# li-kunyi/CUT3R-SLAM

Hardware: AMD Instinct MI355X
Metric: frames/sec (ViT pointmap + covisibility-graph tracking step) on 640x480 (higher is better)
Workload: dtype f16

## Files before the change

cut3r_slam_amd/_lib.py:

```python
from __future__ import annotations

import ctypes as C
import os

_HERE = os.path.dirname(os.path.abspath(__file__))
LIB_PATH = os.path.join(_HERE, "libcut3r_hip.so")

c_void_p, c_int, c_float, c_ll = C.c_void_p, C.c_int, C.c_float, C.c_longlong


class GemmDesc(C.Structure):
    _fields_ = [
        ("A", c_void_p), ("B", c_void_p), ("C", c_void_p), ("bias", c_void_p), ("res1", c_void_p), ("res2", c_void_p),
        ("M", c_int), ("N", c_int), ("K", c_int), ("lda", c_int), ("ldb", c_int), ("ldc", c_int), ("ldr1", c_int),
        ("ldr2", c_int),
        ("act", c_int), ("out_f16", c_int), ("res1_f16", c_int), ("res2_f16", c_int),
        ("batch", c_int),
        ("strideA", c_ll), ("strideB", c_ll), ("strideC", c_ll), ("strideBias", c_ll), ("strideR1", c_ll),
        ("strideR2", c_ll),
        ("conv_k", c_int), ("H", c_int), ("W", c_int), ("Cin", c_int), ("conv_stride", c_int), ("Ho", c_int),
        ("Wo", c_int), ("relu_in", c_int),
        ("shuf", c_int), ("shuf_cout", c_int), ("shuf_Hin", c_int), ("shuf_Win", c_int),
        ("tile", c_int), ("stages", c_int),
        ("rope_pos", c_void_p), ("rope_table", c_void_p), ("rope_cols", c_int), ("rope_pmin", c_int), ("rope_npos", c_int),
        ("rope_d", c_int),
        ("ln_stats", c_void_p), ("ln_colsum", c_void_p), ("ln_nslab", c_int), ("ln_eps", c_float),
        ("stats_out", c_void_p), ("out16", c_void_p), ("ld16", c_int),
    ]


class LcTerm(C.Structure):
    _fields_ = [("a", c_void_p), ("c", c_void_p), ("mask", c_void_p), ("ia", c_int), ("ic", c_int), ("w", c_float), ("pad", c_int)]


SIGNATURES = {
    "cut3r_abi_version": [],
    "cut3r_rope2d": [c_void_p, c_int, c_void_p, c_int, c_int, c_int, c_int, c_ll, c_ll, c_ll, c_float, c_float, c_void_p],
    "cut3r_rope2d_qk": [c_void_p, c_void_p, c_int, c_void_p, c_int, c_int, c_int, c_int, c_ll, c_ll, c_ll, c_ll, c_float, c_float,
                        c_void_p],
    "cut3r_rope2d_tab": [c_void_p, c_void_p, c_ll, c_ll, c_void_p, c_void_p, c_ll, c_ll, c_int, c_int, c_void_p, c_int, c_int, c_float,
                         c_float, c_void_p],
    "cut3r_layernorm": [c_void_p, c_int, c_void_p, c_void_p, c_float, c_int, c_int, c_void_p, c_int, c_void_p, c_int,
                        c_void_p, c_void_p, c_void_p],
    "cut3r_layernorm_dual": [c_void_p, c_int, c_void_p, c_void_p, c_void_p, c_int, c_void_p, c_void_p, c_void_p, c_int, c_float, c_int,
                             c_int, c_void_p],
    "cut3r_layernorm_tokens": [c_void_p, c_int, c_void_p, c_void_p, c_float, c_int, c_int, c_int, c_void_p, c_ll, c_void_p, c_ll, c_void_p,
                               c_ll, c_void_p, c_ll, c_void_p],
    "cut3r_gemm_f16": [C.POINTER(GemmDesc), c_void_p],
    "cut3r_gemm_tile_for": [C.POINTER(GemmDesc)],
    "cut3r_gemm_f16_pair": [C.POINTER(GemmDesc), C.POINTER(GemmDesc), c_void_p],
    "cut3r_gemm_kernel_for": [C.POINTER(GemmDesc)],
    "cut3r_gemm_pair_kernel_for": [C.POINTER(GemmDesc), C.POINTER(GemmDesc)],
    "cut3r_gemm_kernel_count": [],
    "cut3r_rope2d_table": [c_void_p, c_int, c_int, c_int, c_float, c_float, c_void_p],
    "cut3r_gemv_f16w": [c_void_p, c_int, c_void_p, c_int, c_void_p, c_void_p, c_int, c_int, c_int, c_int, c_int,
                        c_void_p, c_int, c_int, c_void_p],
    "cut3r_attention_variant": [c_int],
    "cut3r_attention_kernel_for": [c_int, c_int, c_int, c_int],
    "cut3r_attention_f16": [c_void_p, c_void_p, c_void_p, c_void_p, c_int, c_int, c_int, c_int, c_int,
                            c_ll, c_ll, c_ll, c_ll, c_ll, c_ll, c_ll, c_ll, c_float, c_void_p],
    "cut3r_attention_one_key_f16": [c_void_p, c_void_p, c_int, c_int, c_int, c_int, c_ll, c_ll, c_ll, c_ll, c_void_p],
    "cut3r_im2col_patch": [c_void_p, c_int, c_int, c_int, c_int, c_int, c_int, c_void_p, c_void_p],
    "cut3r_cast_f32_f16": [c_void_p, c_int, c_void_p, c_int, c_int, c_int, c_void_p],
    "cut3r_colmean": [c_void_p, c_int, c_int, c_int, c_void_p, c_void_p],
    "cut3r_colmean_batched": [c_void_p, c_int, c_ll, c_int, c_int, c_int, c_void_p, c_ll, c_void_p],
    "cut3r_upsample2x_nhwc": [c_void_p, c_void_p, c_int, c_int, c_int, c_int, c_void_p],
    "cut3r_dpt_final": [c_void_p, c_int, c_int, c_void_p, c_void_p, c_int, c_void_p, c_void_p, c_void_p],
    "cut3r_conv3x3_dpt_final": [C.POINTER(GemmDesc), c_void_p, c_void_p, c_int, c_void_p, c_ll, c_void_p, c_ll, c_void_p],
    "cut3r_postprocess_pts": [c_void_p, c_int, c_int, c_int, c_void_p, c_void_p, c_void_p],
    "cut3r_postprocess_pose": [c_void_p, c_int, c_void_p, c_void_p],
    "cut3r_patch_overlap": [c_void_p, c_void_p, c_int, c_int, c_float, c_void_p, c_void_p, c_void_p],
    "cut3r_patch_overlap_chain": [c_void_p, c_void_p, c_int, c_int, c_int, c_float, C.c_double, c_void_p, c_void_p, c_void_p, c_void_p,
                                  c_void_p, c_void_p],
    "cut3r_overlap_fwd": [c_void_p, c_int, C.POINTER(c_float), c_float, c_void_p, c_int, c_float, c_float, c_float, c_float,
                          c_int, c_int, c_int, c_void_p, c_void_p],
    "cut3r_overlap_bwd": [c_void_p, c_int, c_int, c_int, c_int, c_void_p, c_float, c_float, c_float, c_float, c_int, c_int,
                          c_void_p, c_void_p],
    "cut3r_window_update": [c_void_p, c_void_p, c_int, c_int, c_int, C.POINTER(c_float), c_float, c_int, c_void_p, c_void_p, c_void_p,
                            c_void_p, c_int, c_int, c_void_p, C.POINTER(c_float), c_int, c_int, c_float, c_float, c_float, c_float,
                            c_void_p, c_int, c_void_p, c_void_p],
    "cut3r_logdepth_accum": [c_void_p, c_void_p, c_int, c_void_p, c_void_p],
    "cut3r_resize_linear_u8": [c_void_p, c_int, c_int, c_int, c_void_p, c_int, c_int, c_int, c_void_p],
    "cut3r_mfma_probe": [c_void_p, c_int, c_int, c_int, c_void_p, c_void_p, c_void_p],
    "cut3r_remap_linear_u8": [c_void_p, c_int, c_int, c_int, c_void_p, c_void_p, c_void_p, c_int, c_int, c_void_p],
    "cut3r_align_view": [c_void_p, c_void_p, c_int, c_int, C.POINTER(c_float), c_float, c_int, c_void_p, c_void_p,
                         c_void_p, c_void_p],
    "cut3r_logdepth_sum": [c_void_p, c_void_p, c_int, c_void_p, c_void_p],
    "cut3r_lie_unary": [c_int, c_int, c_void_p, c_void_p, c_int, c_void_p],
    "cut3r_lie_unary_bwd": [c_int, c_int, c_void_p, c_void_p, c_void_p, c_int, c_void_p],
    "cut3r_lie_mul": [c_int, c_void_p, c_void_p, c_void_p, c_int, c_void_p],
    "cut3r_lie_mul_bwd": [c_int, c_void_p, c_void_p, c_void_p, c_void_p, c_void_p, c_int, c_void_p],
    "cut3r_lie_act": [c_int, c_void_p, c_void_p, c_void_p, c_int, c_int, c_int, c_void_p],
    "cut3r_lie_act_bwd": [c_int, c_void_p, c_void_p, c_void_p, c_void_p, c_void_p, c_int, c_int, c_int, c_void_p],
    "cut3r_lie_adj": [c_int, c_void_p, c_void_p, c_void_p, c_int, c_int, c_void_p],
    "cut3r_lc_workspace_floats": [c_int, c_int],
    "cut3r_lc_optimize": [c_void_p, c_void_p, c_ll, c_void_p, c_void_p, c_void_p, c_int, c_int, c_ll, c_int, c_float,
                          c_void_p, c_void_p, c_void_p, c_void_p, c_void_p, c_void_p, c_void_p],
    "cut3r_lc_optimize_terms": [c_void_p, c_int, c_int, c_int, c_int, c_float, c_void_p, c_void_p, c_void_p, c_void_p, c_void_p, c_void_p,
                                c_void_p],
    "cut3r_lc_optimize_sim3": [c_void_p, c_void_p, c_ll, c_void_p, c_void_p, c_void_p, c_int, c_int, c_ll, c_int, c_float,
                               c_void_p, c_void_p, c_void_p, c_void_p, c_void_p, c_void_p, c_void_p],
    "cut3r_lc_optimize_terms_sim3": [c_void_p, c_int, c_int, c_int, c_int, c_float, c_void_p, c_void_p, c_void_p, c_void_p, c_void_p,
                                     c_void_p, c_void_p],
    "cut3r_transform_submaps": [c_void_p, c_void_p, c_int, c_ll, c_void_p],
    "cut3r_scale_planes": [c_void_p, c_void_p, c_int, c_ll, c_void_p],
    "cut3r_corr_index_forward": [c_void_p, c_void_p, c_void_p, c_int, c_int, c_int, c_int, c_int, c_int, c_void_p],
    "cut3r_corr_index_backward": [c_void_p, c_void_p, c_void_p, c_int, c_int, c_int, c_int, c_int, c_int, c_void_p],
    "cut3r_ba_workspace_floats": [c_int, c_int, c_int, c_int, c_int, c_int],
    "cut3r_ba_assemble": [c_void_p] * 12 + [c_int] * 7 + [c_void_p] * 5,
    "cut3r_ba_solve": [c_void_p, c_void_p, c_void_p, c_int, c_float, c_float, c_void_p, c_void_p, c_void_p, c_void_p],
    "cut3r_ba_backsub": [c_void_p, c_void_p, c_void_p, c_int, c_int, c_int, c_int, c_int, c_int, c_void_p, c_void_p],
    "cut3r_ba_proj_trans": [c_void_p] * 10 + [c_int] * 5 + [c_void_p] * 4,
    "cut3r_bi_inter": [c_void_p, c_void_p, c_int, c_int, c_int, c_int, c_int, c_void_p, c_void_p, c_void_p],
    "cut3r_schur_mono_prior_workspace_floats": [c_int, c_ll],
    "cut3r_schur_mono_prior": [c_void_p] * 5 + [c_int, c_ll, c_float, c_float] + [c_void_p] * 6,
    "cut3r_jdsa_blocks": [c_void_p, c_void_p, c_void_p, c_float, c_int, c_int, c_int, c_void_p, c_void_p, c_void_p, c_void_p],
    "cut3r_depth_filter": [c_void_p] * 5 + [c_int] * 4 + [c_void_p, c_void_p],
    "cut3r_altcorr_forward": [c_void_p, c_void_p, c_void_p] + [c_int] * 8 + [c_void_p, c_void_p],
    "cut3r_altcorr_backward": [c_void_p, c_void_p, c_void_p, c_void_p] + [c_int] * 8 + [c_void_p, c_void_p, c_void_p],
    "cut3r_ba_step": [c_void_p] * 12 + [c_int] * 6 + [c_float, c_float] + [c_void_p] * 5,
    "cut3r_gs_preprocess": [c_int] + [c_void_p] * 5 + [c_int, c_int] + [c_void_p] * 4 + [c_int, c_int] + [c_float] * 4 + [c_void_p] * 5
                           + [c_ll, c_void_p],
    "cut3r_gs_workspace_bytes": [c_int, c_ll],
    "cut3r_gs_bin": [c_int, c_void_p, c_void_p, c_ll, c_int, c_int] + [c_void_p] * 6 + [c_ll, c_void_p, c_void_p],
    "cut3r_gs_render_forward": [c_void_p] * 3 + [c_int, c_int, c_float, c_float] + [c_void_p] * 11,
    "cut3r_pixel_loss_forward": [c_void_p] * 5 + [c_int, c_int] + [c_float] * 4 + [c_void_p, c_void_p],
    "cut3r_pixel_loss_backward": [c_void_p] * 5 + [c_int, c_int] + [c_float] * 4 + [c_void_p] * 4,
    "cut3r_normal_agree_forward": [c_void_p, c_void_p, c_int, c_int] + [c_float] * 4 + [c_void_p, c_void_p],
    "cut3r_normal_agree_backward": [c_void_p, c_void_p, c_int, c_int] + [c_float] * 5 + [c_void_p, c_void_p, c_void_p],
    "cut3r_gs_densify_stats": [c_int] + [c_void_p] * 7,
# ... 126 lines not shown
```

cut3r_slam_amd/csrc/elementwise.hip:

```cpp
#include "common.h"
#include "dpt_tail.h"
#include "../../include/cut3r_hip.h"

namespace {

template <typename T> struct alignas(4 * sizeof(T)) Vec4 { T v[4]; };

template <typename T>
__global__ __launch_bounds__(256) void rope2d_kernel(T* __restrict__ tok, T* __restrict__ tok2, const int64_t* __restrict__ pos,
                                                     int N, int H, int D, long long sB, long long sN, long long sH, long long sB2,
                                                     long long sN2, float base, float fwd) {
    __shared__ float cs[2][2][64];
    const int t = blockIdx.x;
    const int b = t / N, n = t - b * N;
    const int Q = D >> 2;
    if (threadIdx.x < 2 * Q) {
        const int X = threadIdx.x / Q, q = threadIdx.x - X * Q;
        const float inv = fwd / powf(base, (float)q / (float)Q);
        const float fr = (float)pos[(size_t)t * 2 + X] * inv;
        cs[X][0][q] = cosf(fr);
        cs[X][1][q] = sinf(fr);
    }
    __syncthreads();
    const int Q4 = Q >> 2;
// ... 158 lines not shown
        bt[i] = *reinterpret_cast<const f32x4*>(beta + (lane + i * 64) * 4);
    }
    float s = 0.f;
#pragma unroll
    for (int i = 0; i < NV; i++) s += (v[i][0] + v[i][1]) + (v[i][2] + v[i][3]);
    const float mean = wave_sum(s) / (float)C;
    float q = 0.f;
#pragma unroll
    for (int i = 0; i < NV; i++)
#pragma unroll
        for (int e = 0; e < 4; e++) { const float d = v[i][e] - mean; q += d * d; }
    const float rstd = 1.0f / sqrtf(wave_sum(q) / (float)C + eps);
#pragma unroll
    for (int i = 0; i < NV; i++) {
        const int c = (lane + i * 64) * 4;
        f32x4 o;
#pragma unroll
        for (int e = 0; e < 4; e++) o[e] = (v[i][e] - mean) * rstd * g[i][e] + bt[i][e];
        if (mscale) {
            const f32x4 sc = *reinterpret_cast<const f32x4*>(mscale + c);
            const f32x4 sh = *reinterpret_cast<const f32x4*>(mshift + c);
#pragma unroll
            for (int e = 0; e < 4; e++) o[e] = o[e] * (1.0f + sc[e]) + sh[e];
        }
        if (y32r) *reinterpret_cast<f32x4*>(y32r + c) = o;
        if (y16r) {
            const half4_t ho = {(h16)o[0], (h16)o[1], (h16)o[2], (h16)o[3]};
            *reinterpret_cast<half4_t*>(y16r + c) = ho;
        }
    }
}

__global__ __launch_bounds__(256) void layernorm_kernel(const float* __restrict__ x, int ldx, const float* __restrict__ gamma,
                                                        const float* __restrict__ beta, float eps, int M, int C,
                                                        h16* __restrict__ y16, int ld16, float* __restrict__ y32, int ld32,
                                                        const float* __restrict__ mscale, const float* __restrict__ mshift) {
    const int lane = threadIdx.x & 63;
    const int row = blockIdx.x * 4 + (threadIdx.x >> 6);
    if (row >= M) return;
    layernorm_row(x + (size_t)row * ldx, gamma, beta, eps, C, lane, y16 ? y16 + (size_t)row * ld16 : nullptr,
                  y32 ? y32 + (size_t)row * ld32 : nullptr, mscale, mshift);
}

template <int NV>
__global__ __launch_bounds__(256) void layernorm_fast_kernel(const float* __restrict__ x, int ldx, const float* __restrict__ gamma,
                                                             const float* __restrict__ beta, float eps, int M, h16* __restrict__ y16,
                                                             int ld16, float* __restrict__ y32, int ld32,
                                                             const float* __restrict__ mscale, const float* __restrict__ mshift) {
    const int lane = threadIdx.x & 63;
    const int row = blockIdx.x * 4 + (threadIdx.x >> 6);
    if (row >= M) return;
    layernorm_fast_row<NV>(x + (size_t)row * ldx, gamma, beta, eps, lane, y16 ? y16 + (size_t)row * ld16 : nullptr,
                           y32 ? y32 + (size_t)row * ld32 : nullptr, mscale, mshift);
}

struct LnTokDst {
    float* pose32; h16* pose16; h16* tok16; float* tok32;
    long long pose32_gs, pose16_gs, tok16_gs, tok32_gs;
};

template <int NV>
__global__ __launch_bounds__(256) void layernorm_tokens_kernel(const float* __restrict__ x, int ldx, const float* __restrict__ gamma,
                                                               const float* __restrict__ beta, float eps, int M, int C, int N1,
                                                               const LnTokDst d) {
    const int lane = threadIdx.x & 63;
    const int row = blockIdx.x * 4 + (threadIdx.x >> 6);
    if (row >= M) return;
    const int w = row / N1, n = row - w * N1;
    h16* y16r;
    float* y32r;
    if (n == 0) {
        y16r = d.pose16 + (size_t)w * d.pose16_gs;
        y32r = d.pose32 + (size_t)w * d.pose32_gs;
    } else {
        y16r = d.tok16 + (size_t)w * d.tok16_gs + (size_t)(n - 1) * C;
        y32r = d.tok32 ? d.tok32 + (size_t)w * d.tok32_gs + (size_t)(n - 1) * C : nullptr;
    }
    const float* xr = x + (size_t)row * ldx;
    if constexpr (NV > 0) layernorm_fast_row<NV>(xr, gamma, beta, eps, lane, y16r, y32r, nullptr, nullptr);
    else layernorm_row(xr, gamma, beta, eps, C, lane, y16r, y32r, nullptr, nullptr);
}

template <int NV>
__global__ __launch_bounds__(256) void layernorm_dual_kernel(const float* __restrict__ x, int ldx, const float* __restrict__ g1,
                                                             const float* __restrict__ b1, h16* __restrict__ y1, int ld1,
                                                             const float* __restrict__ g2, const float* __restrict__ b2,
                                                             h16* __restrict__ y2, int ld2, float eps, int M) {
    constexpr int C = 256 * NV;
    const int lane = threadIdx.x & 63;
    const int row = blockIdx.x * 4 + (threadIdx.x >> 6);
    if (row >= M) return;
    const float* xr = x + (size_t)row * ldx;
    f32x4 v[NV];
#pragma unroll
    for (int i = 0; i < NV; i++) v[i] = *reinterpret_cast<const f32x4*>(xr + (lane + i * 64) * 4);
    float s = 0.f;
#pragma unroll
    for (int i = 0; i < NV; i++) s += (v[i][0] + v[i][1]) + (v[i][2] + v[i][3]);
    const float mean = wave_sum(s) / (float)C;
    float q = 0.f;
#pragma unroll
    for (int i = 0; i < NV; i++)
#pragma unroll
        for (int e = 0; e < 4; e++) { const float d = v[i][e] - mean; q += d * d; }
    const float rstd = 1.0f / sqrtf(wave_sum(q) / (float)C + eps);
#pragma unroll
    for (int i = 0; i < NV; i++) {
        const int c = (lane + i * 64) * 4;
        const f32x4 ga = *reinterpret_cast<const f32x4*>(g1 + c), ba = *reinterpret_cast<const f32x4*>(b1 + c);
        const f32x4 gb = *reinterpret_cast<const f32x4*>(g2 + c), bb = *reinterpret_cast<const f32x4*>(b2 + c);
        half4_t o1, o2;
#pragma unroll
        for (int e = 0; e < 4; e++) {
            const float n = (v[i][e] - mean) * rstd;
            o1[e] = (h16)(n * ga[e] + ba[e]);
            o2[e] = (h16)(n * gb[e] + bb[e]);
        }
        *reinterpret_cast<half4_t*>(y1 + (size_t)row * ld1 + c) = o1;
        *reinterpret_cast<half4_t*>(y2 + (size_t)row * ld2 + c) = o2;
    }
}

template <bool U8>
__global__ __launch_bounds__(256) void im2col_kernel(const void* __restrict__ img, int B, int C, int H, int W, int P,
                                                     h16* __restrict__ out) {
    const int nh = H / P, nw = W / P;
    const int Kp = C * P * P;
    const size_t total = (size_t)B * nh * nw * (Kp / 8);
    for (size_t i = blockIdx.x * (size_t)blockDim.x + threadIdx.x; i < total; i += (size_t)gridDim.x * blockDim.x) {
        const int kc = (int)(i % (Kp / 8));
        const size_t m = i / (Kp / 8);
        const int k = kc * 8;
        const int c = k / (P * P), rem = k - c * P * P;
        const int iy = rem / P, ix = rem - iy * P;
        const int px = (int)(m % nw);
        const int py = (int)((m / nw) % nh);
        const int b = (int)(m / ((size_t)nw * nh));
        const size_t src = (((size_t)b * C + c) * H + (py * P + iy)) * W + (px * P + ix);
        half8_t o;
        if (U8) {
            const unsigned char* p = (const unsigned char*)img + src;
#pragma unroll
            for (int e = 0; e < 8; e++) o[e] = (h16)(((float)p[e] / 255.0f - 0.5f) / 0.5f);
        } else {
            const float* p = (const float*)img + src;
#pragma unroll
            for (int e = 0; e < 8; e++) o[e] = (h16)p[e];
        }
        *reinterpret_cast<half8_t*>(out + m * Kp + k) = o;
    }
}

__global__ __launch_bounds__(256) void cast_kernel(const float* __restrict__ x, int ldx, h16* __restrict__ y, int ldy, int M, int C4) {
    const size_t total = (size_t)M * C4;
    for (size_t i = blockIdx.x * (size_t)blockDim.x + threadIdx.x; i < total; i += (size_t)gridDim.x * blockDim.x) {
        const int c = (int)(i % C4);
        const size_t m = i / C4;
        f32x4 v = *reinterpret_cast<const f32x4*>(x + m * ldx + c * 4);
        half4_t o = {(h16)v[0], (h16)v[1], (h16)v[2], (h16)v[3]};
        *reinterpret_cast<half4_t*>(y + m * ldy + c * 4) = o;
    }
}

__global__ __launch_bounds__(256) void colmean_kernel(const float* __restrict__ x, int ldx, int M, int C, float* __restrict__ y,
                                                      long long sx, long long sy) {
    __shared__ float part[16][64];
    x += (size_t)blockIdx.y * sx;
    y += (size_t)blockIdx.y * sy;
    const int col = threadIdx.x & 63, rg = threadIdx.x >> 6;
    const int c = blockIdx.x * 64 + col;
    float s0 = 0.f, s1 = 0.f, s2 = 0.f, s3 = 0.f;
    if (c < C) {
        int m = rg;
        for (; m + 12 < M; m += 16) {
            s0 += x[(size_t)m * ldx + c];
            s1 += x[(size_t)(m + 4) * ldx + c];
            s2 += x[(size_t)(m + 8) * ldx + c];
            s3 += x[(size_t)(m + 12) * ldx + c];
        }
        for (; m < M; m += 4) s0 += x[(size_t)m * ldx + c];
    }
    part[rg][col] = (s0 + s1) + (s2 + s3);
    __syncthreads();
    if (rg == 0 && c < C) y[c] = (part[0][col] + part[1][col] + part[2][col] + part[3][col]) / (float)M;
}

__global__ __launch_bounds__(256) void upsample2x_kernel(const h16* __restrict__ in, h16* __restrict__ out, int B, int H, int W, int C8) {
    const int Ho = 2 * H, Wo = 2 * W;
    const float ry = Ho > 1 ? (float)(H - 1) / (float)(Ho - 1) : 0.f;
    const float rx = Wo > 1 ? (float)(W - 1) / (float)(Wo - 1) : 0.f;
    const size_t total = (size_t)B * Ho * Wo * C8;
    for (size_t i = blockIdx.x * (size_t)blockDim.x + threadIdx.x; i < total; i += (size_t)gridDim.x * blockDim.x) {
        const int c = (int)(i % C8);
        size_t p = i / C8;
        const int ox = (int)(p % Wo); p /= Wo;
        const int oy = (int)(p % Ho);
        const int b = (int)(p / Ho);
        const float sy = ry * (float)oy, sx = rx * (float)ox;
        int y0 = (int)sy, x0 = (int)sx;
        const int y1 = y0 + (y0 < H - 1 ? 1 : 0), x1 = x0 + (x0 < W - 1 ? 1 : 0);
        const float ly = sy - (float)y0, lx = sx - (float)x0;
        const float hy = 1.f - ly, hx = 1.f - lx;
        const h16* base = in + (size_t)b * H * W * C8 * 8 + c * 8;
        const half8_t v00 = *reinterpret_cast<const half8_t*>(base + ((size_t)y0 * W + x0) * C8 * 8);
        const half8_t v01 = *reinterpret_cast<const half8_t*>(base + ((size_t)y0 * W + x1) * C8 * 8);
        const half8_t v10 = *reinterpret_cast<const half8_t*>(base + ((size_t)y1 * W + x0) * C8 * 8);
        const half8_t v11 = *reinterpret_cast<const half8_t*>(base + ((size_t)y1 * W + x1) * C8 * 8);
        half8_t o;
#pragma unroll
        for (int e = 0; e < 8; e++)
            o[e] = (h16)(hy * (hx * (float)v00[e] + lx * (float)v01[e]) + ly * (hx * (float)v10[e] + lx * (float)v11[e]));
        *reinterpret_cast<half8_t*>(out + i * 8) = o;
    }
}

DEVINL void act_pts_conf(float x, float y, float z, float c, bool has_conf, bool pos_z, float* pts, float* conf, size_t p) {
    if (pos_z) {
        float sg = (z > 0.f) ? 1.f : ((z < 0.f) ? -1.f : 0.f);
        x *= sg; y *= sg; z *= sg;
    }
    const float d = sqrtf(x * x + y * y + z * z);
    const float dc = fmaxf(d, 1e-8f);
    const float e = expm1f(d);
    pts[3 * p + 0] = x / dc * e;
    pts[3 * p + 1] = y / dc * e;
    pts[3 * p + 2] = z / dc * e;
    if (has_conf) conf[p] = 1.0f + expf(c);
}

__global__ __launch_bounds__(256) void dpt_final_kernel(const h16* __restrict__ in, int P, int Cin, const float* __restrict__ w,
                                                        const float* __restrict__ bsv, int mode, float* __restrict__ pts,
                                                        float* __restrict__ conf) {
    extern __shared__ float sw[];
    const int nout = mode == 0 ? 4 : 3;
    for (int i = threadIdx.x; i < nout * Cin; i += blockDim.x) sw[i] = w[i];
    __syncthreads();
    for (size_t p = blockIdx.x * (size_t)blockDim.x + threadIdx.x; p < (size_t)P; p += (size_t)gridDim.x * blockDim.x) {
        float a0 = bsv[0], a1 = bsv[1], a2 = bsv[2], a3 = nout == 4 ? bsv[3] : 0.f;
        const h16* row = in + p * Cin;
        for (int k = 0; k < Cin; k += 8) {
            half8_t v = *reinterpret_cast<const half8_t*>(row + k);
#pragma unroll
            for (int e = 0; e < 8; e++) {
                const float xv = (float)v[e];
                a0 = fmaf(xv, sw[k + e], a0);
                a1 = fmaf(xv, sw[Cin + k + e], a1);
                a2 = fmaf(xv, sw[2 * Cin + k + e], a2);
                if (nout == 4) a3 = fmaf(xv, sw[3 * Cin + k + e], a3);
            }
        }
        if (mode == 0) {
            dpt_pts_conf<false>(a0, a1, a2, a3, pts + 3 * p, conf + p);
        } else {
            const float eps = 1e-6f;
            float o[3] = {a0, a1, a2};
#pragma unroll
            for (int e = 0; e < 3; e++) {
                float sg = 1.0f / (1.0f + expf(-o[e]));
                pts[3 * p + e] = ((sg * (1 - 2 * eps) + eps) - 0.5f) * 2.0f;
            }
        }
    }
}

__global__ __launch_bounds__(256) void dpt_final_coalesced_kernel(const h16* __restrict__ in, int P, int Cin, const float* __restrict__ w,
                                                                  const float* __restrict__ bsv, int mode, float* __restrict__ pts,
                                                                  float* __restrict__ conf) {
// ... 165 lines not shown
    if (t1 && (!pos1 || ntok1 <= 0)) return CUT3R_ERR_ARG;
    const int Q = D >> 2;
    const int VE = (Q % 8 == 0) ? 8 : 4;
    const long long am = VE - 1;
    if ((stride0 & am) || (t1 && (stride1 & am)) || ((uintptr_t)t0 & (2 * VE - 1)) || (t1 && ((uintptr_t)t1 & (2 * VE - 1)))) return CUT3R_ERR_ARG;
    if (stride0 < (long long)H * D || (t1 && stride1 < (long long)H * D)) return CUT3R_ERR_ARG;
    const long long per_tok = (long long)H * 2 * (Q / VE);
    const long long wa = ntok0 * per_tok, wt = wa + (t1 ? ntok1 * per_tok : 0);
    RopeSeg a{(h16*)t0, pos0, stride0}, b{(h16*)(t1 ? t1 : t0), t1 ? pos1 : pos0, t1 ? stride1 : stride0};
    dim3 grid((unsigned)((wt + 255) / 256)), block(256);
    if (VE == 8)
        hipLaunchKernelGGL((rope2d_tab_kernel<8>), grid, block, 0, (hipStream_t)stream, a, b, wa, wt, H, D, table, pmin, npos, base, fwd);
    else
        hipLaunchKernelGGL((rope2d_tab_kernel<4>), grid, block, 0, (hipStream_t)stream, a, b, wa, wt, H, D, table, pmin, npos, base, fwd);
    return cut3r_check_launch();
}

extern "C" int cut3r_rope2d_qk(void* q, void* k, int dtype, const int64_t* positions, int B, int N, int H, int D, long long q_sB,
                               long long q_sN, long long k_sB, long long k_sN, float base, float fwd, void* stream) {
    if (!k) return CUT3R_ERR_ARG;
    return launch_rope(q, k, dtype, positions, B, N, H, D, q_sB, q_sN, D, k_sB, k_sN, base, fwd, stream);
}

extern "C" int cut3r_layernorm(const float* x, int ldx, const float* gamma, const float* beta, float eps, int M, int C, void* y16,
                               int ld16, float* y32, int ld32, const float* mod_scale, const float* mod_shift, void* stream) {
    if (!x || !gamma || !beta || M <= 0 || C <= 0 || (C & 3) || C > 2048 || (ldx & 3)) return CUT3R_ERR_ARG;
    if (!y16 && !y32) return CUT3R_ERR_ARG;
    if ((y16 && (ld16 & 3)) || (y32 && (ld32 & 3))) return CUT3R_ERR_ARG;
    if ((mod_scale == nullptr) != (mod_shift == nullptr)) return CUT3R_ERR_ARG;
    if (misaligned(x, 15) || misaligned(gamma, 15) || misaligned(beta, 15) || misaligned(y32, 15) || misaligned(y16, 7) ||
        misaligned(mod_scale, 15) || misaligned(mod_shift, 15))
        return CUT3R_ERR_ARG;
    hipStream_t s = (hipStream_t)stream;
    dim3 grid((M + 3) / 4), block(256);
    if (C == 768)
        hipLaunchKernelGGL((layernorm_fast_kernel<3>), grid, block, 0, s, x, ldx, gamma, beta, eps, M, (h16*)y16, ld16, y32, ld32, mod_scale, mod_shift);
    else if (C == 1024)
        hipLaunchKernelGGL((layernorm_fast_kernel<4>), grid, block, 0, s, x, ldx, gamma, beta, eps, M, (h16*)y16, ld16, y32, ld32, mod_scale, mod_shift);
    else if (C == 1536)
        hipLaunchKernelGGL((layernorm_fast_kernel<6>), grid, block, 0, s, x, ldx, gamma, beta, eps, M, (h16*)y16, ld16, y32, ld32, mod_scale, mod_shift);
    else
        hipLaunchKernelGGL(layernorm_kernel, grid, block, 0, s, x, ldx, gamma, beta, eps, M, C, (h16*)y16, ld16, y32, ld32, mod_scale, mod_shift);
    return cut3r_check_launch();
}

extern "C" int cut3r_layernorm_dual(const float* x, int ldx, const float* g1, const float* b1, void* y1, int ld1, const float* g2,
                                    const float* b2, void* y2, int ld2, float eps, int M, int C, void* stream) {
    if (C != 768 && C != 1024 && C != 1536) return CUT3R_ERR_ARG;
    if (!x || !g1 || !b1 || !y1 || !g2 || !b2 || !y2 || M <= 0 || (ldx & 3) || (ld1 & 3) || (ld2 & 3) || !(eps > 0.f)) return CUT3R_ERR_ARG;
    if (misaligned(x, 15) || misaligned(g1, 15) || misaligned(b1, 15) || misaligned(g2, 15) || misaligned(b2, 15) || misaligned(y1, 7) ||
        misaligned(y2, 7))
        return CUT3R_ERR_ARG;
    hipStream_t s = (hipStream_t)stream;
    dim3 grid((M + 3) / 4), block(256);
    if (C == 768) hipLaunchKernelGGL((layernorm_dual_kernel<3>), grid, block, 0, s, x, ldx, g1, b1, (h16*)y1, ld1, g2, b2, (h16*)y2, ld2, eps, M);
    else if (C == 1024) hipLaunchKernelGGL((layernorm_dual_kernel<4>), grid, block, 0, s, x, ldx, g1, b1, (h16*)y1, ld1, g2, b2, (h16*)y2, ld2, eps, M);
    else hipLaunchKernelGGL((layernorm_dual_kernel<6>), grid, block, 0, s, x, ldx, g1, b1, (h16*)y1, ld1, g2, b2, (h16*)y2, ld2, eps, M);
    return cut3r_check_launch();
}

extern "C" int cut3r_layernorm_tokens(const float* x, int ldx, const float* gamma, const float* beta, float eps, int Wn, int N, int C,
                                      float* pose32, long long pose32_gs, void* pose16, long long pose16_gs, void* tok16,
                                      long long tok16_gs, float* tok32, long long tok32_gs, void* stream) {
    if (!x || !gamma || !beta || !pose32 || !pose16 || !tok16 || Wn <= 0 || N <= 0 || C <= 0 || (C & 3) || C > 2048) return CUT3R_ERR_ARG;
    if (ldx < C || (ldx & 3) || !(eps > 0.f)) return CUT3R_ERR_ARG;
    if ((long long)Wn * ((long long)N + 1) > 0x7fffffffLL) return CUT3R_ERR_ARG;
    const long long tok_rows = (long long)N * C;
    if (pose32_gs < C || pose16_gs < C || tok16_gs < tok_rows || (tok32 && tok32_gs < tok_rows)) return CUT3R_ERR_ARG;
    if ((pose32_gs | pose16_gs | tok16_gs | (tok32 ? tok32_gs : 0)) & 3) return CUT3R_ERR_ARG;
    if (misaligned(x, 15) || misaligned(gamma, 15) || misaligned(beta, 15) || misaligned(pose32, 15) || misaligned(tok32, 15) ||
        misaligned(pose16, 7) || misaligned(tok16, 7))
        return CUT3R_ERR_ARG;
    const int M = Wn * (N + 1);
    const LnTokDst d{pose32, (h16*)pose16, (h16*)tok16, tok32, pose32_gs, pose16_gs, tok16_gs, tok32_gs};
    hipStream_t s = (hipStream_t)stream;
    dim3 grid((M + 3) / 4), block(256);
    if (C == 768) hipLaunchKernelGGL((layernorm_tokens_kernel<3>), grid, block, 0, s, x, ldx, gamma, beta, eps, M, C, N + 1, d);
    else if (C == 1024) hipLaunchKernelGGL((layernorm_tokens_kernel<4>), grid, block, 0, s, x, ldx, gamma, beta, eps, M, C, N + 1, d);
    else if (C == 1536) hipLaunchKernelGGL((layernorm_tokens_kernel<6>), grid, block, 0, s, x, ldx, gamma, beta, eps, M, C, N + 1, d);
    else hipLaunchKernelGGL((layernorm_tokens_kernel<0>), grid, block, 0, s, x, ldx, gamma, beta, eps, M, C, N + 1, d);
    return cut3r_check_launch();
}

extern "C" int cut3r_im2col_patch(const void* img, int u8, int B, int C, int H, int W, int P, void* out, void* stream) {
    if (!img || !out || B <= 0 || C <= 0 || P <= 0 || (P & 7) || H % P || W % P) return CUT3R_ERR_ARG;
    const size_t total = (size_t)B * (H / P) * (W / P) * (C * P * P / 8);
    if (u8)
        hipLaunchKernelGGL((im2col_kernel<true>), dim3(grid_for(total)), dim3(256), 0, (hipStream_t)stream, img, B, C, H, W, P, (h16*)out);
    else
        hipLaunchKernelGGL((im2col_kernel<false>), dim3(grid_for(total)), dim3(256), 0, (hipStream_t)stream, img, B, C, H, W, P, (h16*)out);
    return cut3r_check_launch();
}

extern "C" int cut3r_cast_f32_f16(const float* x, int ldx, void* y, int ldy, int M, int C, void* stream) {
    if (!x || !y || M <= 0 || C <= 0 || (C & 3) || (ldx & 3) || (ldy & 3) || misaligned(x, 15) || misaligned(y, 7)) return CUT3R_ERR_ARG;
    hipLaunchKernelGGL(cast_kernel, dim3(grid_for((size_t)M * (C / 4))), dim3(256), 0, (hipStream_t)stream, x, ldx, (h16*)y, ldy, M, C / 4);
    return cut3r_check_launch();
}

extern "C" int cut3r_colmean(const float* x, int ldx, int M, int C, float* y, void* stream) {
    if (!x || !y || M <= 0 || C <= 0) return CUT3R_ERR_ARG;
    hipLaunchKernelGGL(colmean_kernel, dim3((C + 63) / 64), dim3(256), 0, (hipStream_t)stream, x, ldx, M, C, y, 0LL, 0LL);
    return cut3r_check_launch();
}

extern "C" int cut3r_colmean_batched(const float* x, int B, long long stride_x, int ldx, int M, int C, float* y, long long stride_y,
                                     void* stream) {
    if (!x || !y || B <= 0 || B > 65535 || M <= 0 || C <= 0) return CUT3R_ERR_ARG;
    hipLaunchKernelGGL(colmean_kernel, dim3((C + 63) / 64, B), dim3(256), 0, (hipStream_t)stream, x, ldx, M, C, y, stride_x, stride_y);
    return cut3r_check_launch();
}

extern "C" int cut3r_upsample2x_nhwc(const void* in, void* out, int B, int H, int W, int C, void* stream) {
    if (!in || !out || B <= 0 || H <= 0 || W <= 0 || C <= 0 || (C & 7) || misaligned(in, 15) || misaligned(out, 15)) return CUT3R_ERR_ARG;
    const size_t total = (size_t)B * 2 * H * 2 * W * (C / 8);
    hipLaunchKernelGGL(upsample2x_kernel, dim3(grid_for(total)), dim3(256), 0, (hipStream_t)stream, (const h16*)in, (h16*)out, B, H, W, C / 8);
    return cut3r_check_launch();
}

extern "C" int cut3r_dpt_final(const void* in, int P, int Cin, const float* w, const float* b, int mode, float* pts, float* conf,
                               void* stream) {
    if (!in || !w || !b || !pts || P <= 0 || Cin <= 0 || (Cin & 7) || Cin > 2048 || (mode != 0 && mode != 1)) return CUT3R_ERR_ARG;
    if (mode == 0 && !conf) return CUT3R_ERR_ARG;
    if (misaligned(in, 15)) return CUT3R_ERR_ARG;
    const int lpp = Cin / 8;
    if (lpp <= 64 && 64 % lpp == 0) {
        const int ppw = 64 / lpp;
        size_t waves = ((size_t)P + ppw - 1) / ppw;
        size_t blocks = (waves + 3) / 4;
        if (blocks > 8192) blocks = 8192;
        hipLaunchKernelGGL(dpt_final_coalesced_kernel, dim3((unsigned)blocks), dim3(256), 0, (hipStream_t)stream, (const h16*)in, P, Cin, w, b,
                           mode, pts, conf);
    } else {
        hipLaunchKernelGGL(dpt_final_kernel, dim3(grid_for((size_t)P)), dim3(256), 4 * Cin * sizeof(float), (hipStream_t)stream,
                           (const h16*)in, P, Cin, w, b, mode, pts, conf);
    }
    return cut3r_check_launch();
}

extern "C" int cut3r_postprocess_pts(const float* raw, int P, int nch, int pos_z, float* pts, float* conf, void* stream) {
    if (!raw || !pts || P <= 0 || (nch != 3 && nch != 4) || (nch == 4 && !conf)) return CUT3R_ERR_ARG;
    hipLaunchKernelGGL(postprocess_pts_kernel, dim3(grid_for((size_t)P)), dim3(256), 0, (hipStream_t)stream, raw, P, nch, pos_z, pts, conf);
    return cut3r_check_launch();
}

extern "C" int cut3r_postprocess_pose(const float* raw, int B, float* out, void* stream) {
    if (!raw || !out || B <= 0) return CUT3R_ERR_ARG;
    hipLaunchKernelGGL(postprocess_pose_kernel, dim3((B + 63) / 64), dim3(64), 0, (hipStream_t)stream, raw, B, out);
    return cut3r_check_launch();
}

extern "C" int cut3r_resize_linear_u8(const void* src, int H0, int W0, int C, void* dst, int H1, int W1, int chw_out, void* stream) {
    if (!src || !dst || H0 < 1 || W0 < 1 || H1 < 1 || W1 < 1 || C < 1 || C > 4 || H1 > 65535) return CUT3R_ERR_ARG;
    hipLaunchKernelGGL(resize_linear_u8_kernel, dim3((W1 + 255) / 256, H1), dim3(256), 0, (hipStream_t)stream,
                       (const unsigned char*)src, H0, W0, C, (unsigned char*)dst, H1, W1, chw_out);
    return cut3r_check_launch();
}

extern "C" int cut3r_remap_linear_u8(const void* src, int H, int W, int C, const int32_t* map_ix, const int32_t* map_iy, void* dst, int Ho,
                                     int Wo, void* stream) {
    if (!src || !dst || !map_ix || !map_iy || H < 1 || W < 1 || Ho < 1 || Wo < 1 || C < 1 || C > 4 || Ho > 65535) return CUT3R_ERR_ARG;
    hipLaunchKernelGGL(remap_linear_u8_kernel, dim3((Wo + 255) / 256, Ho), dim3(256), 0, (hipStream_t)stream, (const unsigned char*)src, H, W,
                       C, map_ix, map_iy, (unsigned char*)dst, Ho, Wo);
    return cut3r_check_launch();
}
```

cut3r_slam_amd/dist.py:

```python
from __future__ import annotations

import contextlib
import os
import time
from typing import Callable, List, Sequence, Tuple

import torch
import torch.distributed as dist


def window_ranges(first_t0: int, count: int, win: int = 5) -> List[Tuple[int, int]]:
    return [(first_t0 + win * j, first_t0 + win * j + win + 1) for j in range(count)]


def all_gather_outputs(outs: Sequence[torch.Tensor], world: int, force_collective: bool = False) -> List[torch.Tensor]:
    if not dist.is_initialized() or (world == 1 and not force_collective):
        return [t.clone() for t in outs]
    res = []
    for t in outs:
        t = t.contiguous()
        if t.is_cuda and dist.get_backend() == "nccl":
            buf = torch.empty((world,) + tuple(t.shape), dtype=t.dtype, device=t.device)
            dist.all_gather_into_tensor(buf.view(-1), t.view(-1))
        else:
            parts = [torch.empty_like(t) for _ in range(world)]
            dist.all_gather(parts, t)
            buf = torch.stack(parts, 0)
        res.append(buf.reshape((world * t.shape[0],) + tuple(t.shape[1:])))
    return res


def memory_plan(world: int, steps: int, wb: int = 28, H: int = 384, W: int = 512, win: int = 5, ds: int = 2, feat_dim: int = 1024, patch: int = 16,
                weights_bytes: int = 1_610_000_000, workspace_bytes: int = 0, frames_resident: int = 2000, frame_bytes: int = 480 * 640 * 3,
                hbm_bytes: int = 288 * 10**9):
    n_kf = 7 + win * wb * world * steps + 2 + 8
    nsub = n_kf // win + 1
    h, w = H // ds, W // ds
    tokens = (H // patch) * (W // patch)
    feat_rows = max(64, 2 * (win * wb * world + 1)) + 6
    plan = {
        "keyframes": n_kf,
        "image_u8": n_kf * 3 * H * W,
        "depth_f32": n_kf * H * W * 4,
        "submap_ds_f32": nsub * (win + 1) * h * w * 3 * 4,
        "conf_ds_f32": nsub * (win + 1) * h * w * 4,
        "w2c_f32": n_kf * 12 * 4,
        "encoder_feature_ring_f32": feat_rows * tokens * feat_dim * 4,
        "camera_frames_u8": frames_resident * frame_bytes,
        "weights_f16": int(weights_bytes),
        "network_workspaces": int(workspace_bytes),
    }
    plan["total"] = sum(v for k, v in plan.items() if k != "keyframes")
    plan["hbm"] = int(hbm_bytes)
    plan["fits"] = plan["total"] <= 0.9 * hbm_bytes
    return plan


class PinnedFrames:

    def __init__(self, host_frames: torch.Tensor, virtual_len: int, device, ring: int = 16, upload_every_frame: bool = False):
        assert not host_frames.is_cuda and host_frames.dtype == torch.uint8 and host_frames.dim() == 4
        self.base = host_frames if host_frames.is_pinned() else host_frames.pin_memory()
        self.period = self.base.shape[0]
        self.shape = (int(virtual_len),) + tuple(self.base.shape[1:])
        self.device, self.dtype, self.is_cuda = torch.device(device), torch.uint8, False
        self.stream = torch.cuda.Stream(device=self.device)
        self.ring = torch.empty((int(ring),) + tuple(self.base.shape[1:]), dtype=torch.uint8, device=self.device)
        self._slot = 0
        self.upload_every_frame = bool(upload_every_frame)
        self._uploaded_upto = 0
        self._scratch = None
        self.bytes_uploaded = 0

    def fetch(self, f: int) -> torch.Tensor:
        slot = self._slot
        self._slot = (slot + 1) % self.ring.shape[0]
        dst = self.ring[slot:slot + 1]
        with torch.cuda.stream(self.stream):
            dst.copy_(self.base[int(f) % self.period][None], non_blocking=True)
        self.bytes_uploaded += dst.numel()
        return dst

    def upload_range(self, a: int, b: int, keep: Callable[[int], bool]):
        if not self.upload_every_frame:
            return
        if self._scratch is None:
            self._scratch = torch.empty((32,) + tuple(self.base.shape[1:]), dtype=torch.uint8, device=self.device)
        cap = self._scratch.shape[0]
        with torch.cuda.stream(self.stream):
            f = max(a, self._uploaded_upto)
            while f < b:
                if keep(f):
                    f += 1
                    continue
                g = f + 1
                while g < b and not keep(g) and g - f < cap and (g % self.period) > (f % self.period):
                    g += 1
                src = self.base[f % self.period:f % self.period + (g - f)]
                self._scratch[:g - f].copy_(src, non_blocking=True)
                self.bytes_uploaded += src.numel()
                f = g
        self._uploaded_upto = max(self._uploaded_upto, b)

    def event(self) -> torch.cuda.Event:
        ev = torch.cuda.Event()
        ev.record(self.stream)
        return ev

    def __getitem__(self, key):
        if isinstance(key, slice):
            a = 0 if key.start is None else key.start
            b = self.shape[0] if key.stop is None else key.stop
            return torch.stack([self.base[f % self.period] for f in range(a, b)], 0).to(self.device)
        return self.base[int(key) % self.period].to(self.device)


class ShardedTracker:

    def __init__(self, slam, world: int, rank: int, wb: int = 1, infer_fn: Callable = None, track_fn: Callable = None,
                 append_fn: Callable = None, pipelined: bool = True, views: int = 6, force_collective: bool = False):
        self.slam, self.world, self.rank, self.wb = slam, world, rank, max(1, int(wb))
        self.infer_fn = infer_fn
        self.track_fn = track_fn
        self.append_fn = append_fn or self._append
        self.pipelined = pipelined
        self.views = views
        self.force_collective = force_collective
        self.emulate_gather = False
        self.shard_counting = os.environ.get("CUT3R_SHARD_COUNTING", "1") == "1"
        self._pending = None
        self._next_t0 = None
        self._side = None
        self._pose_pinned = [None, None]
        self._appended_upto = 0
        self._enc_stream, self._ahead = None, None
        self.encode_ahead = os.environ.get("CUT3R_ENC_AHEAD", "1") == "1"
        self.side_priority = int(os.environ.get("CUT3R_SIDE_PRIORITY", "0"))
        self.scan = world > 1 or force_collective or os.environ.get("CUT3R_SCAN", "0") == "1"
        self.replicate_depth = os.environ.get("CUT3R_REPLICATE_DEPTH", "0") == "1"
        self._chain = None
        self._f0 = 0
        self._upload_ev = None
        slam.tracked_only = True
        self.stats = {"append_s": 0.0, "issue_s": 0.0, "issue_enc_s": 0.0, "replay_s": 0.0, "replay_wait_s": 0.0, "exchange_s": 0.0, "steps": 0}

    def frames_needed(self, total_steps: int, kf_every: int, win: int) -> int:
        return (7 + win * self.world * self.wb * total_steps + 1) * kf_every + 1

    def _append(self, kf_index: int, frame, tstamp, intr, mine: bool):
        kf = self.slam.keyframes
        if mine and frame is not None and frame.dim() == 4 and frame.shape[-1] == 3 and frame.shape[1] != 3:
            from . import ops
            i = kf.counter.value
            kf.append(tstamp, None, None, None, None, None, intr, None, None)
            ops.resize_linear_u8(frame[0], kf.ht, kf.wd, chw_out=True, out=kf.image[i])
            return
        kf.append(tstamp, frame[0] if (mine and frame is not None) else None, None, None, None, None, intr, None, None)

    def _encode(self, ranges):
        tr = self.slam.tracker
        if self.world > 1:
            self.slam.keyframes.feat_valid[ranges[0][0]] = False
        tr.window_features(ranges[0][0], ranges[-1][1])
        return torch.stack([tr.window_features(a, b) for a, b in ranges], 0)

    def _decode(self, feats):
        kf = self.slam.keyframes
        res = self.slam.model.decode_windows(feats, kf.ht, kf.wd)
        return tuple(res[k] for k in ("pts3d_in_self_view", "conf_self", "camera_pose"))

    def _side_ctx(self, gathered, ev):
        if ev is None or not self.pipelined:
            return contextlib.nullcontext()
        if self._side is None:
            self._side = self._make_side_stream()
        return torch.cuda.stream(self._side)

    def _make_side_stream(self):
        self._skipped = [torch.cuda.Stream() for _ in range(int(os.environ.get("CUT3R_SIDE_SKIP", "0")))]
        return torch.cuda.Stream(priority=self.side_priority)

    def _exchange_counts(self, counts):
        if self.emulate_gather or not dist.is_initialized():
            return counts
        if dist.get_backend() == "nccl":
            dev = counts.cuda(non_blocking=True)
            dist.all_reduce(dev, op=dist.ReduceOp.SUM)
            return dev.cpu()
        dist.all_reduce(counts, op=dist.ReduceOp.SUM)
        return counts

    def _replay(self, pending, defer=False):
        fin = None
        ranges_all, gathered, ev = pending
        V = self.views
        tic = time.perf_counter()
        if ev is not None and self.pipelined:
            if self._side is None:
                self._side = self._make_side_stream()
            self._side.wait_event(ev)
            ev.synchronize()
            self.stats["replay_wait_s"] += time.perf_counter() - tic
            for g in (gathered if not self.scan or self.track_fn is not None else [t for o in gathered[0] for t in o]):
                if torch.is_tensor(g) and g.is_cuda:
                    g.record_stream(self._side)
            ctx = torch.cuda.stream(self._side)
        else:
            if ev is not None:
                ev.synchronize()
                self.stats["replay_wait_s"] += time.perf_counter() - tic
            ctx = contextlib.nullcontext()
        with ctx:
            if self.scan and self.track_fn is None:
                fin = self._replay_scan(ranges_all, gathered, defer)
                self.slam.tracker.t1 = ranges_all[-1][1]
                self.stats["replay_s"] += time.perf_counter() - tic
                return fin
            outs = [tuple(g[j * V:(j + 1) * V] for g in gathered) for j in range(len(ranges_all))]
            if self.track_fn is not None:
                for (a, b), o in zip(ranges_all, outs):
                    self.track_fn(a, b, o)
                    self.slam.tracker.t1 = b
            else:
                mask, exch = None, None
                if (self.world > 1 or self.force_collective) and self.shard_counting:
                    mask = [self.rank * self.wb <= j < (self.rank + 1) * self.wb for j in range(len(ranges_all))]
                    exch = self._exchange_counts
                fin = self.slam.tracker.track_many(ranges_all, outs, count_mask=mask, exchange=exch, defer_decisions=defer)
                self.slam.tracker.t1 = ranges_all[-1][1]
        self.stats["replay_s"] += time.perf_counter() - tic
        return fin

    def _gather_rows(self, block, per_rank):
        world, rank = self.world, self.rank
        if self.emulate_gather:
            own = block[rank * per_rank:(rank + 1) * per_rank]
            for r in range(world):
                if r != rank:
                    block[r * per_rank:(r + 1) * per_rank].copy_(own)
            return
        if not dist.is_initialized() or (world == 1 and not self.force_collective):
            return
        if block.is_cuda and dist.get_backend() == "nccl":
            own = block[rank * per_rank:(rank + 1) * per_rank]
            dist.all_gather_into_tensor(block.view(-1), own.reshape(-1))
        else:
            own = block[rank * per_rank:(rank + 1) * per_rank].cpu()
            parts = [torch.empty_like(own) for _ in range(world)]
            dist.all_gather(parts, own)
            for r in range(world):
                if r != rank:
# ... 6 lines not shown
            self._gather_rows(kf.conf_ds[sub0:sub0 + n], self.wb)
        elif self.replicate_depth:
            self._gather_rows(kf.depth[sub0 * 5:(sub0 + n) * 5], self.wb * 5)

    def _replay_scan(self, ranges_all, payload, defer):
        own_outs, scal = payload
        tr = self.slam.tracker
        if self._chain is None:
            self._chain = tr.chain_state(ranges_all[0][0])
        i0 = self.rank * self.wb
        return tr.track_sharded(ranges_all, (i0, i0 + self.wb), own_outs, scal.numpy(), self._chain, self._gather_store,
                                self._exchange_counts, defer_decisions=defer)

    def _exchange_scalars(self, scal_own):
        world = self.world
        if self.emulate_gather:
            return torch.cat([scal_own] * world, 0)
        if not dist.is_initialized() or (world == 1 and not self.force_collective):
            return scal_own
        if scal_own.is_cuda and dist.get_backend() == "nccl":
            buf = torch.empty((world,) + tuple(scal_own.shape), dtype=scal_own.dtype, device=scal_own.device)
            dist.all_gather_into_tensor(buf.view(-1), scal_own.reshape(-1))
            return buf.view(-1, scal_own.shape[1])
        host = scal_own.cpu()
        parts = [torch.empty_like(host) for _ in range(world)]
        dist.all_gather(parts, host)
        return torch.cat(parts, 0).to(scal_own.device)

    def _append_range(self, frames, t, n_frames, kf_every, win, intr, first_t0):
        slam, world, rank, wb = self.slam, self.world, self.rank, self.wb
        host = isinstance(frames, PinnedFrames)
        if host:
            frames.upload_range(max(t, self._appended_upto), t + n_frames, lambda f: f % kf_every == 0)
        ctx = torch.cuda.stream(frames.stream) if host else contextlib.nullcontext()
        with ctx:
            self._append_frames(frames, t, n_frames, kf_every, win, intr, host)
        if host:
            self._upload_ev = frames.event()
        self._appended_upto = max(self._appended_upto, t + n_frames)

    def _append_frames(self, frames, t, n_frames, kf_every, win, intr, host):
        slam, world, rank, wb = self.slam, self.world, self.rank, self.wb
        for f in range(max(t, self._appended_upto), t + n_frames):
            if f % kf_every == 0:
                k = slam.keyframes.counter.value
                o = k - self._f0
                blk = (o - 1) // (win * wb) if o >= 1 else 0
                mine = blk % world == rank or (o >= 1 and o % (win * wb) == 0 and (blk + 1) % world == rank)
                self.append_fn(k, (frames.fetch(f) if host else frames[f:f + 1]) if mine else None, f, intr, mine)

    def step(self, frames, t, kf_every, win, intr):
        slam, world, rank, wb = self.slam, self.world, self.rank, self.wb
        if not getattr(slam.keyframes, "calibrated", True):
            raise RuntimeError("ShardedTracker needs a calibrated keyframe store: multi-GPU self-calibration is not supported, pass intrinsics")
        if self._next_t0 is None:
            self._next_t0 = slam.tracker.t1 - 1
            self._f0 = self._next_t0
        first_t0 = self._next_t0
        ranges_all = window_ranges(first_t0, world * wb, win)
        mine = ranges_all[rank * wb:(rank + 1) * wb]
        n_frames = world * wb * win * kf_every
        tic0 = time.perf_counter()
        self._append_range(frames, t, n_frames, kf_every, win, intr, first_t0)
        tic = time.perf_counter()
        self.stats["append_s"] += tic - tic0
        if self.infer_fn is not None:
            outs = self.infer_fn(mine)
            self.stats["issue_s"] += time.perf_counter() - tic
            if self._pending is not None:
                self._replay(self._pending)
                self._pending = None
        else:
            if self._ahead is not None and self._ahead[0] == mine:
                _, feats, ev_enc = self._ahead
                torch.cuda.current_stream().wait_event(ev_enc)
                feats.record_stream(torch.cuda.current_stream())
            else:
                if self._ahead is not None:
                    torch.cuda.current_stream().wait_event(self._ahead[2])
                if self._upload_ev is not None:
                    torch.cuda.current_stream().wait_event(self._upload_ev)
                feats = self._encode(mine)
            self._ahead = None
            self.stats["issue_s"] += time.perf_counter() - tic
            self.stats["issue_enc_s"] += time.perf_counter() - tic
            t_next = t + n_frames
            if self.encode_ahead and self.pipelined and t_next + n_frames <= frames.shape[0] and feats.is_cuda:
                nxt_first = ranges_all[-1][1] - 1
                nxt_all = window_ranges(nxt_first, world * wb, win)
                nxt_mine = nxt_all[rank * wb:(rank + 1) * wb]
                self._append_range(frames, t_next, n_frames, kf_every, win, intr, nxt_first)
                if self._enc_stream is None:
                    self._enc_stream = torch.cuda.Stream()
                self._enc_stream.wait_stream(torch.cuda.current_stream())
                if self._upload_ev is not None:
                    self._enc_stream.wait_event(self._upload_ev)
                with torch.cuda.stream(self._enc_stream):
                    nf = self._encode(nxt_mine)
                    ev_enc = torch.cuda.Event()
                    ev_enc.record()
                self._ahead = (nxt_mine, nf, ev_enc)
            fin = None
            if self._pending is not None:
                fin = self._replay(self._pending, defer=True)
                self._pending = None
            tic = time.perf_counter()
            outs = self._decode(feats)
            self.stats["issue_s"] += time.perf_counter() - tic
            if fin is not None:
                tic = time.perf_counter()
                fin()
                self.stats["replay_s"] += time.perf_counter() - tic
        if self.scan and self.infer_fn is None:
            tic = time.perf_counter()
            V = self.views
            own = [tuple(o[j * V:(j + 1) * V].clone() for o in outs) for j in range(wb)]
            scal = self._exchange_scalars(slam.tracker.window_scalars(own))
            slot = self.stats["steps"] & 1
            if self._pose_pinned[slot] is None or self._pose_pinned[slot].shape != scal.shape or self._pose_pinned[slot].dtype != scal.dtype:
                self._pose_pinned[slot] = torch.empty(tuple(scal.shape), dtype=scal.dtype).pin_memory()
            scal_host = self._pose_pinned[slot]
            scal_host.copy_(scal, non_blocking=True)
            ev = torch.cuda.Event()
            ev.record()
            self.stats["exchange_s"] += time.perf_counter() - tic
            self.stats["steps"] += 1
            self._pending = (ranges_all, (own, scal_host), ev)
            self._next_t0 = ranges_all[-1][1] - 1
            if not self.pipelined:
                self.flush()
            return t + n_frames
        tic = time.perf_counter()
        if self.emulate_gather:
            gathered = [torch.cat([t] * world, 0) for t in outs]
        else:
            gathered = all_gather_outputs(outs, world, self.force_collective)
        self.stats["exchange_s"] += time.perf_counter() - tic
        self.stats["steps"] += 1
        ev = None
        if gathered[0].is_cuda:
            slot = self.stats["steps"] & 1
            if self._pose_pinned[slot] is None or self._pose_pinned[slot].shape != gathered[2].shape:
                self._pose_pinned[slot] = torch.empty(gathered[2].shape, dtype=gathered[2].dtype).pin_memory()
            pose_host = self._pose_pinned[slot]
            pose_host.copy_(gathered[2], non_blocking=True)
            gathered = [gathered[0], gathered[1], pose_host]
            ev = torch.cuda.Event()
            ev.record()
        self._pending = (ranges_all, gathered, ev)
        self._next_t0 = ranges_all[-1][1] - 1
        if not self.pipelined:
            self.flush()
        return t + n_frames

    def flush(self):
        if self._pending is not None:
            self._replay(self._pending)
            self._pending = None
        if self._side is not None:
            torch.cuda.current_stream().wait_stream(self._side)
```

cut3r_slam_amd/keyframe.py:

```python
from __future__ import annotations

import numpy as np
import torch

from . import geom_host as gh


class _FeatValid:

    def __init__(self, buffer, rows):
        self.rows = rows
        self.flags = [False] * buffer if not rows else None
        self.tags = [-1] * rows if rows else None

    def __getitem__(self, i):
        return self.flags[i] if self.flags is not None else self.tags[i % self.rows] == i

    def __setitem__(self, i, v):
        if self.flags is not None:
            self.flags[i] = bool(v)
        elif v:
            self.tags[i % self.rows] = i
        elif self.tags[i % self.rows] == i:
            self.tags[i % self.rows] = -1


class KeyFrame:
    def __init__(self, config, image_size, buffer, downsample_ratio, device="cuda:0", feat_dim=1024, patch=16, feat_buffer=0):
        self.ht = ht = int(image_size[0])
        self.wd = wd = int(image_size[1])
        self.buffer = int(buffer)
        self.is_initialized = False
        self.config = config
        self.downsample_ratio = ds = int(downsample_ratio)
        self.device = torch.device(device)
        self._counter = 0
        dev = self.device
        self.tstamp = torch.zeros(buffer, dtype=torch.float)
        self.image = torch.zeros(buffer, 3, ht, wd, device=dev, dtype=torch.uint8)
        self.intrinsic = torch.zeros(buffer, 4, dtype=torch.float)
        self.calibrated = False
        self.pose = torch.zeros(buffer, 7, dtype=torch.float)
        self.pose[:] = torch.as_tensor([0, 0, 0, 0, 0, 0, 1], dtype=torch.float)
        self.w2c = torch.zeros(buffer, 12, device=dev, dtype=torch.float)
        nsub = buffer // 5 + 1
        self.submap_ds = torch.ones(nsub, 6, ht // ds, wd // ds, 3, device=dev, dtype=torch.float)
        self.conf_ds = torch.zeros(nsub, 6, ht // ds, wd // ds, device=dev, dtype=torch.float)
        self.depth = torch.ones(buffer, ht, wd, device=dev, dtype=torch.float)
        n = (ht // patch) * (wd // patch)
        self.feat_rows = int(feat_buffer) if 0 < int(feat_buffer) < buffer else 0
        self.featI = torch.zeros(self.feat_rows + 6 if self.feat_rows else buffer, n, feat_dim, dtype=torch.float, device=dev)
        self.pos = torch.zeros(buffer if not self.feat_rows else 1, n, 2, dtype=torch.int64, device=dev)
        self.feat_valid = _FeatValid(buffer, self.feat_rows)

    def feat_store(self, a: int, b: int, feats) -> None:
        R = self.feat_rows
        if not R:
            self.featI[a:b] = feats
        else:
            if b - a > R:
                raise ValueError("feature ring smaller than one encoder batch")
            i = a
            while i < b:
                r = i % R
                m = min(b - i, R - r)
                self.featI[r:r + m] = feats[i - a:i - a + m]
                if r < 6:
                    k = min(m, 6 - r)
                    self.featI[R + r:R + r + k] = feats[i - a:i - a + k]
                i += m
        for i in range(a, b):
            self.feat_valid[i] = True

    def feat_slice(self, t0: int, t1: int):
        R = self.feat_rows
        if not R:
            return self.featI[t0:t1]
        if t1 - t0 > 6:
            raise ValueError("feature ring: windows of at most 6 keyframes")
        r = t0 % R
        return self.featI[r:r + (t1 - t0)]

    class _Counter:
        def __init__(self, kf):
            self._kf = kf

        @property
        def value(self):
            return self._kf._counter

        @value.setter
        def value(self, v):
            self._kf._counter = int(v)

    @property
    def counter(self):
        return KeyFrame._Counter(self)

    def set_pose(self, index: int, pose7) -> None:
        p = torch.as_tensor(np.asarray(pose7, np.float32))
        self.pose[index] = p
        rows = gh.w2c_rows(gh.pose_vec_to_matrix(p.numpy()[None]))
        self.w2c[index].copy_(torch.from_numpy(rows[0]), non_blocking=True)

    def set_poses(self, start: int, poses7, upload: bool = True) -> np.ndarray:
        p = np.asarray(poses7, np.float32).reshape(-1, 7)
        n = p.shape[0]
        self.pose[start:start + n] = torch.from_numpy(p)
        rows = gh.w2c_rows(gh.pose_vec_to_matrix(p))
        if upload:
            self.w2c[start:start + n].copy_(torch.from_numpy(rows), non_blocking=True)
        return rows

    def set_poses_at(self, idx, poses7):
        p = np.asarray(poses7, np.float32).reshape(-1, 7)
        rows = gh.w2c_rows(gh.pose_vec_to_matrix(p))
        for j, k in enumerate(idx):
            self.pose[int(k)] = torch.from_numpy(p[j])
            self.w2c[int(k)].copy_(torch.from_numpy(rows[j]))

    def set_intrinsics(self, K) -> None:
        k4 = torch.as_tensor(K, dtype=torch.float).reshape(-1)[:4]
        self.intrinsic[:max(self._counter, 1)] = k4
        self.calibrated = True

    def pointmap_slot(self, kf: int, sub_num: int, t0: int):
        if kf >= t0:
            return sub_num, kf - t0
        return kf // 5, kf % 5

    def append(self, tstamp, image, pose, _unused, depth, normal, intrinsics, feat=None, pos=None):
        i = self._counter
        if i >= self.buffer:
            raise IndexError(f"keyframe buffer overflow ({self.buffer}); raise --buffer")
        self._counter = i + 1
        self.tstamp[i] = float(tstamp)
        if image is not None:
            self.image[i].copy_(image.to(self.device, non_blocking=True))
        if pose is not None:
            self.set_pose(i, pose)
        if depth is not None:
            self.depth[i].copy_(torch.as_tensor(depth).to(self.device))
        if intrinsics is not None:
            self.intrinsic[i] = torch.as_tensor(intrinsics, dtype=torch.float).reshape(-1)[:4]
            self.calibrated = True
        else:
            self.intrinsic[i] = self.intrinsic[0].clone()
        if feat is not None:
            self.feat_store(i, i + 1, feat[None] if feat.dim() == 2 else feat)
        if pos is not None and not self.feat_rows:
            self.pos[i].copy_(pos.reshape(self.pos[i].shape))
```

cut3r_slam_amd/model.py:

```python
from __future__ import annotations

import contextlib
import gc
import math
import os
import re
from dataclasses import dataclass, field
from typing import Dict, List, NamedTuple, Optional

import torch

from . import ops
from .config import Cut3rConfig, production_config, state_dict_schema

F16, F32 = torch.float16, torch.float32


def _env_flag(name: str, default: bool) -> bool:
    return os.environ.get(name, "1" if default else "0") != "0"


def _env_int(name: str, default: int) -> int:
    return int(os.environ.get(name, str(default)))


@dataclass
class ARCroco3DStereoOutput:
    ress: Optional[List[dict]] = None
    views: Optional[List[dict]] = None


class _Lin:

    def __init__(self, w: torch.Tensor, b: Optional[torch.Tensor], dev):
        n = w.shape[0]
        self.n = n
        pad = (-n) % 4
        w2 = w.reshape(n, -1).to(F32)
        if pad:
            w2 = torch.cat([w2, torch.zeros(pad, w2.shape[1])], 0)
            if b is not None:
                b = torch.cat([b.to(F32), torch.zeros(pad)], 0)
        self.w = w2.to(device=dev, dtype=F16).contiguous()
        self.b = b.to(device=dev, dtype=F32).contiguous() if b is not None else None
        self.npad = n + pad
        self.k = self.w.shape[1]


class _Stream(NamedTuple):
    x: torch.Tensor
    x16: Optional[torch.Tensor] = None
    st: Optional[torch.Tensor] = None


@dataclass
class _Block:
    p: str
    tag: str
    x: _Stream
    y: _Stream
    out: _Stream
    xpos: Optional[torch.Tensor]
    ypos: Optional[torch.Tensor]
    heads: int
    B: int
    pre_ln: bool = False
    C: int = field(init=False)
    Nx: int = field(init=False)
    Ny: int = field(init=False)
    D: int = field(init=False)
    fold_x: bool = field(init=False, default=False)
    fold_y: bool = field(init=False, default=False)
    fold_o: bool = field(init=False, default=False)
    emit: Optional[tuple] = field(init=False, default=None)
    ln16: Optional[torch.Tensor] = field(init=False, default=None)
    y16: Optional[torch.Tensor] = field(init=False, default=None)
    qkv: Optional[torch.Tensor] = field(init=False, default=None)
    attn: Optional[torch.Tensor] = field(init=False, default=None)
    q: Optional[torch.Tensor] = field(init=False, default=None)
    kv: Optional[torch.Tensor] = field(init=False, default=None)
    cattn: Optional[torch.Tensor] = field(init=False, default=None)
    mlp_h: Optional[torch.Tensor] = field(init=False, default=None)

    def __post_init__(self):
        self.C = self.x.x.shape[1]
        self.Nx, self.Ny, self.D = self.x.x.shape[0] // self.B, self.y.x.shape[0] // self.B, self.C // self.heads


class Cut3rModel:
    def __init__(self, cfg: Cut3rConfig, state_dict: Dict[str, torch.Tensor], device="cuda:0", minimal: bool = False):
        self.cfg = cfg
        self.device = torch.device(device)
        self.minimal = minimal
        schema = state_dict_schema(cfg)
        missing = [k for k in schema if k not in state_dict]
        if missing:
            raise KeyError(f"state_dict is missing {len(missing)} tensors, e.g. {missing[:4]}")
        for k, shp in schema.items():
            if tuple(state_dict[k].shape) != tuple(shp):
                raise ValueError(f"{k}: shape {tuple(state_dict[k].shape)} != schema {tuple(shp)}")
        self._buf: Dict[tuple, torch.Tensor] = {}
        self._graphs: Dict[tuple, tuple] = {}
        self.use_graphs = _env_flag("CUT3R_GRAPHS", True)
        self.dual_stream = _env_flag("CUT3R_DUAL_STREAM", True)
        self.dual_ln = _env_flag("CUT3R_DUAL_LN", True)
        self.pair_gemm = _env_flag("CUT3R_PAIR_GEMM", False)
        self.pair_rows = _env_int("CUT3R_PAIR_ROWS", 0)
        self.fused_rope = _env_int("CUT3R_FUSED_ROPE", 1)
        self.rope48_rows = _env_int("CUT3R_ROPE48_ROWS", 0)
        self.head_overlap = _env_flag("CUT3R_HEAD_OVERLAP", True)
        self.dpt_fuse = _env_flag("CUT3R_DPT_FUSE", True)
        self.head_chunk = max(1, _env_int("CUT3R_HEAD_CHUNK", 28))
        self.one_key = _env_flag("CUT3R_ONE_KEY", True)
        self.ln_fold = _env_int("CUT3R_LN_FOLD", 1)
        self._head_stream = None
        self._side = None
        self._head_side = None
        self._enc_last = None
        self._enc_events: Dict[int, torch.cuda.Event] = {}
        self._prep(state_dict)

    @classmethod
    def from_state_dict(cls, cfg, sd, device="cuda:0", **kw):
        return cls(cfg, sd, device, **kw)

    @classmethod
    def from_pretrained(cls, path: str, config: Optional[Cut3rConfig] = None, device="cuda:0", **kw):
        import argparse
        if not os.path.isfile(path):
            raise FileNotFoundError(f"{path}: no checkpoint (this runtime never fetches from a hub)")
        with torch.serialization.safe_globals([argparse.Namespace]):
            ckpt = torch.load(path, map_location="cpu", weights_only=True)
        sd = ckpt["model"] if "model" in ckpt else ckpt
        sd = {(k[7:] if k.startswith("module.") else k): v for k, v in sd.items()}
        if not any(k.startswith("dec_blocks_state") for k in sd):
            for k in list(sd):
                if k.startswith("dec_blocks"):
                    sd[k.replace("dec_blocks", "dec_blocks_state")] = sd[k]
        if config is None:
            config = production_config()
            args = getattr(ckpt.get("args", None), "model", "") if isinstance(ckpt, dict) else ""
            config = _config_from_ctor_string(args, config)
        return cls(config, sd, device, **kw)

    def to(self, device):
        return self

    def eval(self):
        return self

    def _prep(self, sd):
        cfg, dev = self.cfg, self.device
        f32 = lambda k: sd[k].to(device=dev, dtype=F32).contiguous()
        self.w: Dict[str, object] = {}

        def lin(name, key=None):
            key = key or name
            self.w[name] = _Lin(sd[key + ".weight"], sd.get(key + ".bias"), dev)

        def ln(name):
            self.w[name] = (f32(name + ".weight"), f32(name + ".bias"))

        def fold(name, w, b, norm):
            if not self.ln_fold or w.shape[1] % 64 or w.shape[0] % 4 or w.shape[1] > ops.LN_FOLD_MAX_K:
                return
            gam, bet = sd[norm + ".weight"].double(), sd[norm + ".bias"].double()
            wd = w.double()
            L = _Lin((wd * gam[None, :]).float(), None, dev)
            L.b = (wd @ bet + b.double()).to(device=dev, dtype=F32).contiguous()
            L.c = L.w.double().sum(1).to(F32).contiguous()
            self.w[name + "@ln"] = L

        def enc_block(p):
            ln(p + ".norm1"); lin(p + ".attn.qkv"); lin(p + ".attn.proj"); ln(p + ".norm2")
            lin(p + ".mlp.fc1"); lin(p + ".mlp.fc2")
            if self.ln_fold >= 2:
                fold(p + ".attn.qkv", sd[p + ".attn.qkv.weight"], sd[p + ".attn.qkv.bias"], p + ".norm1")
                fold(p + ".mlp.fc1", sd[p + ".mlp.fc1.weight"], sd[p + ".mlp.fc1.bias"], p + ".norm2")

        def dec_block(p, folded=True):
            ln(p + ".norm1"); lin(p + ".attn.qkv"); lin(p + ".attn.proj")
            ln(p + ".norm2"); ln(p + ".norm3"); ln(p + ".norm_y")
            lin(p + ".cross_attn.projq"); lin(p + ".cross_attn.proj")
            wkv = torch.cat([sd[p + ".cross_attn.projk.weight"], sd[p + ".cross_attn.projv.weight"]], 0)
            bkv = torch.cat([sd[p + ".cross_attn.projk.bias"], sd[p + ".cross_attn.projv.bias"]], 0)
            self.w[p + ".cross_attn.projkv"] = _Lin(wkv, bkv, dev)
            lin(p + ".mlp.fc1"); lin(p + ".mlp.fc2")
            if folded:
                fold(p + ".attn.qkv", sd[p + ".attn.qkv.weight"], sd[p + ".attn.qkv.bias"], p + ".norm1")
                fold(p + ".cross_attn.projq", sd[p + ".cross_attn.projq.weight"], sd[p + ".cross_attn.projq.bias"], p + ".norm2")
                fold(p + ".cross_attn.projkv", wkv, bkv, p + ".norm_y")
                fold(p + ".mlp.fc1", sd[p + ".mlp.fc1.weight"], sd[p + ".mlp.fc1.bias"], p + ".norm3")

        self.w["patch_embed"] = _Lin(sd["patch_embed.proj.weight"], sd["patch_embed.proj.bias"], dev)
        for i in range(cfg.enc_depth):
            enc_block(f"enc_blocks.{i}")
        ln("enc_norm")
# ... 85 lines not shown

    def _linear(self, x16, name, out, act=0, res1=None, res2=None, skinny=False, rope=None, ln=None, emit=None, cols=None):
        L, rope, ln = self._panel(name, rope, ln)
        w, b = L.w, L.b
        if cols is not None:
            assert skinny and rope is None and ln is None and emit is None, "a column range: the skinny kernel only"
            w, b = w[cols[0]:cols[1]], (b[cols[0]:cols[1]] if b is not None else None)
        return ops.linear(x16, w, out, b, act, res1, res2, tile=16 if skinny else 0, rope=rope, ln=ln, emit=emit)

    def _project(self, probs, act=0):
        if not probs:
            return None
        if len(probs) == 1:
            return self._linear(act=act, **probs[0])

        def prob(x16, name, out, res1=None, skinny=False, rope=None, ln=None, emit=None):
            assert not skinny, "the pair kernels have no one-row-per-sequence form"
            L, rope, ln = self._panel(name, rope, ln)
            return (x16, L.w, out, L.b, res1, dict(rope=rope, ln=ln, emit=emit))
        ops.linear_pair(prob(**probs[0]), prob(**probs[1]), act)

    def _folded(self, name):
        return self.ln_fold and (name + "@ln") in self.w

    def _xs(self, tag, x):
        M, Cc = x.shape
        return self.buf(tag + ".x16", (M, Cc), F16), self.buf(tag + ".xst", (Cc // 64, M, 2), F32)

    def _fuse_rope(self, pos, D, rows):
        dims = (64, 48) if (self.fused_rope == 2 or (self.fused_rope and rows <= self.rope48_rows)) else (64,)
        return self.fused_rope and pos is not None and D in dims and pos.is_contiguous() and pos.numel() == 2 * rows

    def _ln(self, x, name, out16=None, out32=None, mod=None):
        g, b = self.w[name]
        ops.layernorm(x, g, b, self.cfg.ln_eps, out16, out32, mod[0] if mod else None, mod[1] if mod else None)

    def _rope(self, t, pos):
        ops.rope_2d_pair(t, pos, None, None, self.cfg.rope_freq, 1.0)

    def _self_attn(self, tag, x_ln16, B, N, heads, pos, p, out, res, ln=None, emit=None):
        Cc = x_ln16.shape[1]
        D = Cc // heads
        sk = N == 1
        qkv = self.buf(tag + ".qkv", (B * N, 3 * Cc), F16)
        fuse = (not sk) and self._fuse_rope(pos, D, B * N)
        self._linear(x_ln16, p + ".qkv", qkv, skinny=sk, rope=(pos, 2 * Cc, D) if fuse else None, ln=ln)
        v5 = qkv.view(B, N, 3, heads, D)
        q, k, v = v5[:, :, 0], v5[:, :, 1], v5[:, :, 2]
        if pos is not None and not fuse:
            ops.rope_2d_pair(q, pos, k, pos, self.cfg.rope_freq, 1.0)
        a = self.buf(tag + ".attn", (B, N, heads, D), F16)
        ops.attention(q, k, v, a, D ** -0.5)
        self._linear(a.view(B * N, Cc), p + ".proj", out, res1=res, skinny=sk, emit=emit)

    def _mlp(self, tag, x_ln16, p, out, res, ln=None, emit=None):
        M = x_ln16.shape[0]
        hdim = self.w[p + ".fc1"].npad
        h = self.buf(tag + ".mlp_h", (M, hdim), F16)
        self._linear(x_ln16, p + ".fc1", h, act=1, ln=ln)
        self._linear(h, p + ".fc2", out, res1=res, emit=emit)

    @contextlib.contextmanager
    def _encoder_turn(self):
        if torch.cuda.is_current_stream_capturing():
            yield
            return
        cur = torch.cuda.current_stream()
        last = self._enc_last
        if last is not None and last[0] != cur:
            cur.wait_event(last[1])
        try:
            yield
        finally:
            ev = self._enc_events.get(cur.cuda_stream)
            if ev is None:
                ev = self._enc_events[cur.cuda_stream] = torch.cuda.Event()
            ev.record(cur)
            self._enc_last = (cur, ev)

    def _encode(self, img: torch.Tensor):
        with self._encoder_turn():
            return self._encode_pass(img)

    def _encode_pass(self, img: torch.Tensor):
        cfg = self.cfg
        B, _, H, W = img.shape
        P, E = cfg.patch_size, cfg.enc_embed_dim
        nh, nw = H // P, W // P
        N = nh * nw
        M = B * N
        tag = f"enc{B}x{N}"
        patches = self.buf(tag + ".patches", (M, 3 * P * P), F16)
        ops.im2col_patch(img.contiguous(), P, patches)
        x = self.buf(tag + ".x", (M, E), F32)
        self._linear(patches, "patch_embed", x)
        y, xx = torch.meshgrid(torch.arange(nh, device=self.device), torch.arange(nw, device=self.device), indexing="ij")
        pos = torch.stack([y.reshape(-1), xx.reshape(-1)], -1)[None].expand(B, -1, -1).contiguous()
        ln16 = self.buf(tag + ".ln16", (M, E), F16)
        fold = self.ln_fold >= 2 and self._folded("enc_blocks.0.attn.qkv") and E % 64 == 0
        x16, xst = self._xs(tag, x) if fold else (None, None)
        em = (xst, x16) if fold else None
        for i in range(cfg.enc_depth):
            p = f"enc_blocks.{i}"
            if fold and i > 0:
                self._self_attn(tag, x16, B, N, cfg.enc_num_heads, pos, p + ".attn", x, x, ln=xst, emit=em)
            else:
                self._ln(x, p + ".norm1", out16=ln16)
                self._self_attn(tag, ln16, B, N, cfg.enc_num_heads, pos, p + ".attn", x, x, emit=em)
            if fold:
                self._mlp(tag, x16, p + ".mlp", x, x, ln=xst, emit=em if i + 1 < cfg.enc_depth else None)
            else:
                self._ln(x, p + ".norm2", out16=ln16)
                self._mlp(tag, ln16, p + ".mlp", x, x)
        feat = torch.empty((B, N, E), dtype=F32, device=self.device)
        feat16 = torch.empty((B, N, E), dtype=F16, device=self.device)
        self._ln(x, "enc_norm", out16=feat16.view(M, E), out32=feat.view(M, E))
        return feat, feat16, pos

    def _graphed(self, kind, fn, inp):
        key = (kind, tuple(inp.shape), inp.dtype)
        ent = self._graphs.get(key)
        if ent is None:
            static_in = inp.clone()
            cur = torch.cuda.current_stream()
            side = torch.cuda.Stream()
            side.wait_stream(cur)
            with torch.cuda.stream(side):
                for _ in range(2):
                    fn(static_in)
            cur.wait_stream(side)
            torch.cuda.synchronize()
            graph = torch.cuda.CUDAGraph()
            gc_was_on = gc.isenabled()
            gc.collect()
            gc.disable()
            try:
                with torch.cuda.graph(graph):
                    out = fn(static_in)
            finally:
                if gc_was_on:
                    gc.enable()
            ent = (graph, static_in, out)
            self._graphs[key] = ent
        graph, static_in, out = ent
        static_in.copy_(inp, non_blocking=True)
        graph.replay()
        return out

    def normalize(self, img_tensor):
        return (img_tensor / 255.0 - 0.5) / 0.5

    def encode_image(self, view):
        img = view["img"]
        if not img.is_cuda:
            img = img.to(self.device)
        B = img.shape[0]
        im_shape = view.get("true_shape", torch.tensor(img.shape[-2:])[None].repeat(B, 1))
        img = img.to(F32) if img.dtype != torch.uint8 else img
        if self.use_graphs:
            with self._encoder_turn():
                feat, _, pos = self._graphed("enc", self._encode, img.contiguous())
                feat = feat.clone()
        else:
            feat, _, pos = self._encode(img)
        return feat, pos, im_shape

    def _block(self, p, tag, x, y, out, xpos, ypos, heads, B=1, fresh=False, pre_ln=False):
        s = _Block(p, tag, x, y, out, xpos, ypos, heads, B, pre_ln)
        C, Nx, Ny, D = s.C, s.Nx, s.Ny, s.D
        can = lambda t, n, name: bool(t.x16 is not None and n > 1 and self._folded(p + name))
        s.fold_x = fresh and can(x, Nx, ".attn.qkv")
        s.fold_y = fresh and can(y, Ny, ".cross_attn.projkv")
        s.fold_o = can(out, Nx, ".mlp.fc1")
        s.emit = (out.st, out.x16) if s.fold_o else None
        s.ln16 = self.buf(tag + ".ln16", (B * Nx, C), F16)
        s.y16 = self.buf(tag + ".y16", (B * Ny, C), F16)
        s.qkv = self.buf(tag + ".qkv", (B * Nx, 3 * C), F16)
        s.attn = self.buf(tag + ".attn", (B, Nx, heads, D), F16)
        s.q = self.buf(tag + ".q", (B, Nx, heads, D), F16)
        s.kv = self.buf(tag + ".kv", (B * Ny, 2 * C), F16)
        s.cattn = self.buf(tag + ".cattn", (B, Nx, heads, D), F16)
        s.mlp_h = self.buf(tag + ".mlp_h", (B * Nx, self.w[p + ".mlp.fc1"].npad), F16)
        return s

    def _pair_carries(self, rows):
        return rows <= self.pair_rows

    def _dec_layer(self, blocks, fork=False):
        pair = len(blocks) == 2
        assert not pair or all(s.Nx > 1 and s.Ny > 1 for s in blocks), "pair launches need more than one row per sequence"
        carry = pair and self._pair_carries(max(s.B * max(s.Nx, s.Ny) for s in blocks))
        assert not pair or carry or not any(s.fold_x or s.fold_y or s.fold_o for s in blocks), "the plain pair kernels take no LayerNorm fold"
        fuse = lambda s, pos, n: bool(n > 1 and self._fuse_rope(pos, s.D, s.B * n) and (not pair or (carry and s.D == 64)))
        fuse_x, fuse_y = (lambda s: fuse(s, s.xpos, s.Nx)), (lambda s: fuse(s, s.ypos, s.Ny))

        def each(fn, need=lambda s: True):
            todo = [s for s in blocks if need(s)]
            if fork and len(todo) == 2:
                cur = torch.cuda.current_stream()
                self._side.wait_stream(cur)
                with torch.cuda.stream(self._side):
                    fn(todo[0])
                fn(todo[1])
                cur.wait_stream(self._side)
            else:
                for s in todo:
                    fn(s)

        rows = lambda t: t.view(-1, t.shape[-2] * t.shape[-1])
        skx, sky = (lambda s: s.Nx == 1), (lambda s: s.Ny == 1)
        one_x, one_y = (lambda s: self.one_key and s.Nx == 1), (lambda s: self.one_key and s.Ny == 1)
        each(lambda s: self._ln(s.x.x, s.p + ".norm1", out16=s.ln16), lambda s: not (s.fold_x or s.pre_ln))
        self._project([dict(x16=s.x.x16 if s.fold_x else s.ln16, name=s.p + ".attn.qkv", out=s.qkv, skinny=skx(s),
                            rope=(s.xpos, 2 * s.C, s.D) if fuse_x(s) else None, ln=s.x.st if s.fold_x else None)
                       if not one_x(s) else
                       dict(x16=s.ln16, name=s.p + ".attn.qkv", out=rows(s.attn), skinny=True, cols=(2 * s.C, 3 * s.C)) for s in blocks])

        def self_attn(s):
            v5 = s.qkv.view(s.B, s.Nx, 3, s.heads, s.D)
            q, k, v = v5[:, :, 0], v5[:, :, 1], v5[:, :, 2]
            if s.xpos is not None and not fuse_x(s):
                ops.rope_2d_pair(q, s.xpos, k, s.xpos, self.cfg.rope_freq, 1.0)
            ops.attention(q, k, v, s.attn, s.D ** -0.5)
        each(self_attn, lambda s: not one_x(s))
        self._project([dict(x16=rows(s.attn), name=s.p + ".attn.proj", out=s.out.x, res1=s.x.x, skinny=skx(s), emit=s.emit) for s in blocks])
        each(lambda s: self._ln(s.out.x, s.p + ".norm2", out16=s.ln16), lambda s: not (s.fold_o or one_y(s)))
        self._project([dict(x16=s.out.x16 if s.fold_o else s.ln16, name=s.p + ".cross_attn.projq", out=rows(s.q), skinny=skx(s),
                            rope=(s.xpos, s.C, s.D) if fuse_x(s) else None, ln=s.out.st if s.fold_o else None) for s in blocks if not one_y(s)])
# ... 73 lines not shown
        if x.is_contiguous():
            ops.linear(x.view(-1, Cc), L.w, out.view(-1, L.npad), L.b)
        else:
            ops.linear_batched(x.view(B, H * W, Cc), L.w.unsqueeze(0).expand(B, -1, -1), out.view(B, H * W, L.npad),
                               None if L.b is None else L.b.unsqueeze(0).expand(B, -1))
        return out

    def _convT(self, x, name):
        L = self.w[name]
        B, H, W, Cc = x.shape
        cout = L.npad // (L.s * L.s)
        out = self.buf(name, (B, H * L.s, W * L.s, cout), F16)
        return ops.conv_transpose_nhwc(x, L.w, out, L.b, L.s)

    def _up2(self, x, tag):
        B, H, W, Cc = x.shape
        return ops.upsample2x(x, self.buf(tag, (B, 2 * H, 2 * W, Cc), F16))

    def _rcu(self, x, p, res2=None):
        t = self._conv3(x, p + ".conv1", relu_in=True, act=2)
        return self._conv3(t, p + ".conv2", res1=x, res2=res2)

    def _fusion(self, p, x0, x1=None):
        out = x0 if x1 is None else self._rcu(x1, p + ".resConfUnit1", res2=x0)
        out = self._rcu(out, p + ".resConfUnit2")
        out = self._up2(out, p + ".up")
        return self._conv1(out, p + ".out_conv")

    def _dpt(self, p, toks16: List[torch.Tensor], B, nh, nw, last=True):
        a = p + ".act_postprocess"
        t = [x.view(B, nh, nw, -1) for x in toks16]
        l0 = self._convT(self._conv1(t[0], a + ".0.0"), a + ".0.1")
        l1 = self._convT(self._conv1(t[1], a + ".1.0"), a + ".1.1")
        l2 = self._conv1(t[2], a + ".2.0")
        l3 = self._conv3(self._conv1(t[3], a + ".3.0"), a + ".3.1", stride=2)
        L = [self._conv3(l, f"{p}.scratch.layer_rn.{i}") for i, l in enumerate((l0, l1, l2, l3))]
        p4 = self._fusion(p + ".scratch.refinenet4", L[3])
        if p4.shape[1] != L[2].shape[1] or p4.shape[2] != L[2].shape[2]:
            p4 = p4[:, : L[2].shape[1], : L[2].shape[2]].contiguous()
        p3 = self._fusion(p + ".scratch.refinenet3", p4, L[2])
        p2 = self._fusion(p + ".scratch.refinenet2", p3, L[1])
        p1 = self._fusion(p + ".scratch.refinenet1", p2, L[0])
        o = self._conv3(p1, p + ".head.0")
        o = self._up2(o, p + ".head.up")
        if last:
            o = self._conv3(o, p + ".head.2", act=2)
        return o

    def _dpt_fused(self, p):
        L = self.w[p + ".head.2"]
        return self.dpt_fuse and L.b is not None and ops.conv3x3_dpt_final_ok(L.w.shape[1] // 9, L.npad, self.w[p + ".head.4.w"])

    def _dpt_pts(self, p, toks16, B, nh, nw, H, W, key_pts, key_conf, res, out=None):
        fused = self._dpt_fused(p)
        o = self._dpt(p, toks16, B, nh, nw, last=not fused)
        if out is None:
            pts = torch.empty((B, H, W, 3), dtype=F32, device=self.device)
            conf = torch.empty((B, H, W), dtype=F32, device=self.device)
        else:
            pts, conf = out
        if fused:
            L = self.w[p + ".head.2"]
            ops.conv3x3_dpt_final(o, L.w, L.b, self.w[p + ".head.4.w"], self.w[p + ".head.4.b"], pts, conf)
        else:
            ops.dpt_final(o.view(B * H * W, -1), self.w[p + ".head.4.w"], self.w[p + ".head.4.b"], 0, pts, conf)
        if res is not None:
            res[key_pts], res[key_conf] = pts, conf

    @torch.no_grad()
    def forward_window(self, imgs: torch.Tensor, return_taps: bool = False):
        if self.use_graphs and not return_taps:
            with self._encoder_turn():
                return self._graphed("win", lambda x: self._forward_window(x, False), imgs.contiguous())
        return self._forward_window(imgs, return_taps)

    @torch.no_grad()
    def encode_batch(self, imgs: torch.Tensor) -> torch.Tensor:
        if self.use_graphs:
            with self._encoder_turn():
                feat, _, _ = self._graphed("enc", self._encode, imgs.contiguous())
                return feat.clone()
        return self._encode(imgs)[0]

    @torch.no_grad()
    def decode_window(self, feats: torch.Tensor, H: int, W: int):
        if self.use_graphs:
            return self._graphed(("dec", H, W), lambda f: self._forward_window(None, False, feats=f, hw=(H, W)), feats.contiguous())
        return self._forward_window(None, False, feats=feats, hw=(H, W))

    def _forward_window(self, imgs, return_taps: bool = False, feats=None, hw=None):
        P = self.cfg.patch_size
        if feats is None:
            V, _, H, W = imgs.shape
            feat, feat16, _ = self._encode(imgs)
            res, taps = self._decode(feat[None], feat16[None], H, W, return_taps)
        else:
            H, W = hw
            res, taps = self._decode(feats[None], None, H, W, return_taps)
            V = feats.shape[0]
        preds = [{k: v[i:i + 1] for k, v in res.items()} for i in range(V)]
        return preds, taps

    @torch.no_grad()
    def decode_windows(self, feats: torch.Tensor, H: int, W: int):
        if self.use_graphs:
            return self._graphed(("decW", H, W), lambda f: self._decode(f, None, H, W, False)[0], feats.contiguous())
        return self._decode(feats, None, H, W, False)[0]

    def _decode(self, feat, feat16, H, W, return_taps=False):
        cfg = self.cfg
        P, E, D, Ld = cfg.patch_size, cfg.enc_embed_dim, cfg.dec_embed_dim, cfg.dec_depth
        Wn, V, N, _ = feat.shape
        nh, nw = H // P, W // P
        S = cfg.state_size
        dev = self.device
        if feat16 is None:
            feat16 = self.buf("win.feat16", (Wn, V, N, E), F16)
            ops.cast_f16(feat.reshape(Wn * V * N, E), feat16.view(Wn * V * N, E))
        y, xx = torch.meshgrid(torch.arange(nh, device=dev), torch.arange(nw, device=dev), indexing="ij")
        pos1 = torch.stack([y.reshape(-1), xx.reshape(-1)], -1)[None]
        pos_img = torch.cat([-torch.ones(1, 1, 2, dtype=torch.int64, device=dev), pos1], dim=1).expand(Wn, -1, -1).contiguous()
        pos_state = self.state_pos.expand(Wn, -1, -1).contiguous()
        taps = {"enc_feat": feat[0]} if return_taps else None

        small = self._pair_carries(Wn * max(N + 1, S))
        pair = self.pair_gemm or small
        fold = self.ln_fold and D % 64 == 0 and self._folded("dec_blocks.0.attn.qkv") and (small or not pair)

        def stream(name, rows):
            x = self.buf(name, (rows, D), F32)
            return _Stream(x, *self._xs(name, x)) if fold else _Stream(x)
        st = [stream("dec.state0", Wn * S), stream("dec.state1", Wn * S)]
        im = [stream("dec.img0", Wn * (N + 1)), stream("dec.img1", Wn * (N + 1))]
        s0 = self.buf("dec.s0", (S, D), F32)
        self._linear(self.register_tokens16, "decoder_embed_state", s0)
        st[0].x.view(Wn, S, D).copy_(s0[None].expand(Wn, -1, -1))
        msz = self.mem0.shape[0]
        mem = [self.buf("dec.mem0", (Wn * msz, 2 * D), F32), self.buf("dec.mem1", (Wn * msz, 2 * D), F32)]
        mem[0].view(Wn, msz, 2 * D).copy_(self.mem0[None].expand(Wn, -1, -1))
        h1, h2 = Ld * 2 // 4, Ld * 3 // 4
        tok1 = self.buf("head.tok1", (Wn, V, N, D), F16)
        tok2 = self.buf("head.tok2", (Wn, V, N, D), F16)
        tok3 = self.buf("head.tok3", (Wn, V, N, D), F16)
        tok3_32 = self.buf("head.tok3_32", (Wn, V, N, D), F32) if not self.minimal else None
        pose_tok = self.buf("head.pose_tok", (Wn, V, D), F32)
        pose_tok16 = self.buf("head.pose_tok16", (Wn, V, D), F16)
        g32 = self.buf("dec.g32", (Wn, E), F32)
        g16 = self.buf("dec.g16", (Wn, E), F16)
        if not self.one_key:
            dn32 = self.buf("dec.dn32", (Wn * (N + 1), D), F32)
            dn16 = self.buf("dec.dn16", (Wn * (N + 1), D), F16)
        Lde = self.w["decoder_embed"]
        w_de = Lde.w.unsqueeze(0).expand(Wn, -1, -1)
        b_de = Lde.b.unsqueeze(0).expand(Wn, -1)
        states = []
        cs, cm = 0, 0
        fork = self.dual_stream and self.use_graphs and torch.cuda.is_current_stream_capturing()
        if fork and self._side is None:
            self._side = torch.cuda.Stream()
        head_fork = fork and self.head_overlap and cfg.head_type == "dpt"
        head_pts = head_conf = None
        if head_fork:
            if self._head_stream is None:
                self._head_stream = torch.cuda.Stream()
            head_pts = torch.empty((Wn * V, H, W, 3), dtype=F32, device=dev)
            head_conf = torch.empty((Wn * V, H, W), dtype=F32, device=dev)
        for i in range(V):
            ops.colmean_batched(feat[:, i], g32)
            ops.cast_f16(g32, g16)
            a, b = im[0], im[1]
            a3 = a.x.view(Wn, N + 1, D)
            if i == 0:
                a3[:, 0] = self.pose_token
            else:
                a3[:, 0] = self._mem_inquire(g16, mem[cm], Wn)
            ops.linear_batched(feat16[:, i], w_de, a3[:, 1:], b_de)
            s_a, s_b = st[cs], st[cs ^ 1]
            dead_tail = (i == V - 1) and not return_taps
            fresh = False
            for l in range(Ld):
                last = dead_tail and l == Ld - 1
                pre = bool(not last and self.dual_ln and D in (768, 1024, 1536) and not (fold and fresh))
                if pre:
                    self._dual_norms(l, a.x, s_a.x)
                image = self._block(f"dec_blocks.{l}", "deci", a, s_a, b, pos_img, pos_state, cfg.dec_num_heads, Wn, fresh, pre)
                state = None if last else self._block(f"dec_blocks_state.{l}", "decs", s_a, a, s_b, pos_state, pos_img, cfg.state_dec_num_heads,
                                                      Wn, fresh, pre)
                if last:
                    self._dec_layer([image])
                elif pair:
                    self._dec_layer([state, image], fork)
                elif fork:
                    cur = torch.cuda.current_stream()
                    self._side.wait_stream(cur)
                    with torch.cuda.stream(self._side):
                        self._dec_layer([state])
                    self._dec_layer([image])
                    cur.wait_stream(self._side)
                else:
                    self._dec_layer([state])
                    self._dec_layer([image])
                s_a, s_b = s_b, s_a
                a, b = b, a
                fresh = True
                for tk, h in ((tok1, h1), (tok2, h2)):
                    if l + 1 == h:
                        tk[:, i].copy_(a.x.view(Wn, N + 1, D)[:, 1:])
            if not dead_tail:
                self._ln(s_a.x, "dec_norm_state", out32=s_b.x)
            new_state = s_b
            if self.one_key:
                ops.layernorm_tokens(a.x, *self.w["dec_norm"], cfg.ln_eps, pose_tok[:, i], pose_tok16[:, i], tok3[:, i],
                                     None if tok3_32 is None else tok3_32[:, i])
            else:
                self._ln(a.x, "dec_norm", out16=dn16, out32=dn32)
                dn16v, dn32v = dn16.view(Wn, N + 1, D), dn32.view(Wn, N + 1, D)
                tok3[:, i].copy_(dn16v[:, 1:])
                if tok3_32 is not None:
                    tok3_32[:, i].copy_(dn32v[:, 1:])
                pose_tok[:, i].copy_(dn32v[:, 0])
                pose_tok16[:, i].copy_(dn16v[:, 0])
            if not dead_tail:
                self._mem_update(mem[cm], g16, pose_tok[:, i], mem[cm ^ 1], Wn)
                cm ^= 1
            if head_fork:
                cur = torch.cuda.current_stream()
                self._head_stream.wait_stream(cur)
                with torch.cuda.stream(self._head_stream):
                    for c0 in range(0, Wn, self.head_chunk):
                        c1 = min(Wn, c0 + self.head_chunk)
                        nb = c1 - c0
                        tk = []
                        for name, src, dim in (("f", feat16, E), ("t1", tok1, D), ("t2", tok2, D), ("t3", tok3, D)):
                            if self.one_key:
                                tk.append(src[c0:c1, i])
                                continue
                            t = self.buf("head.view." + name, (nb, N, dim), F16)
                            t.copy_(src[c0:c1, i])
                            tk.append(t.view(nb * N, dim))
                        pd, cd = head_pts.view(Wn, V, H, W, 3)[c0:c1, i], head_conf.view(Wn, V, H, W)[c0:c1, i]
                        if self._dpt_fused("downstream_head.dpt_self"):
                            self._dpt_pts("downstream_head.dpt_self", tk, nb, nh, nw, H, W, None, None, None, out=(pd, cd))
                        else:
                            pv = self.buf("head.view.pts", (nb, H, W, 3), F32)
                            cv = self.buf("head.view.conf", (nb, H, W), F32)
                            self._dpt_pts("downstream_head.dpt_self", tk, nb, nh, nw, H, W, None, None, None, out=(pv, cv))
                            pd.copy_(pv)
                            cd.copy_(cv)
            cs = 0 if new_state is st[0] else 1
            if return_taps:
                states.append((new_state.x.view(Wn, S, D)[0].clone(), mem[cm].view(Wn, msz, 2 * D)[0].clone()))
        if return_taps:
# ... 141 lines not shown
```

cut3r_slam_amd/ops.py:

```python
from __future__ import annotations

import ctypes as C
import os
from typing import Optional

import torch

from . import _lib, views
from ._lib import GemmDesc, check

F16, F32 = torch.float16, torch.float32


def _stream():
    return C.c_void_p(torch.cuda.current_stream().cuda_stream)


def _p(t: Optional[torch.Tensor]):
    return C.c_void_p(t.data_ptr()) if t is not None else C.c_void_p(0)


def _req(cond, msg):
    if not cond:
        raise ValueError(msg)
# ... 72 lines not shown
    if pos.shape != (B, N, 2) or pos.dtype != torch.int64 or not pos.is_contiguous() or not pos.is_cuda:
        raise RuntimeError("positions must be contiguous int64 [B,N,2]")
    return _p(t), _p(pos), B * N, t.stride(1)


def rope_2d_pair(t0, pos0, t1, pos1, base, fwd=1.0):
    H, D = t0.shape[2:]
    if D % 16 != 0:
        raise RuntimeError("cut3r_slam_amd.rope_2d: head dims that are multiples of 16 only (CUT3R uses 16/32/48/64)")
    if not _ROPE_TABLE_LAUNCH:
        if t1 is not None and pos1 is pos0 and t1.shape == t0.shape:
            return rope_2d_qk(t0, t1, pos0, base, fwd)
        rope_2d(t0, pos0, base, fwd)
        if t1 is not None:
            rope_2d(t1, pos1, base, fwd)
        return
    if t1 is not None and tuple(t1.shape[2:]) != (H, D):
        raise RuntimeError("rope_2d_pair: both tensors must have the same heads and head dim")
    a = _rope_seg(t0, pos0)
    b = _rope_seg(t1, pos1) if t1 is not None else (None, None, 0, 0)
    tab = rope_table(t0.device, base, fwd, D)
    lib = _lib.load()
    check(lib.cut3r_rope2d_tab(a[0], a[1], a[2], a[3], b[0], b[1], b[2], b[3], H, D, _p(tab), ROPE_PMIN, ROPE_NPOS, float(base), float(fwd),
                               _stream()), "cut3r_rope2d_tab")


def layernorm(x, gamma, beta, eps=1e-6, out16=None, out32=None, mod_scale=None, mod_shift=None):
    _cuda(x, gamma, beta, out16, out32, mod_scale, mod_shift)
    _req(x.dtype == F32 and x.dim() == 2 and x.stride(1) == 1, "x must be fp32 [M,C] with unit inner stride")
    M, Cc = x.shape
    _req(gamma.dtype == F32 and beta.dtype == F32 and gamma.numel() == Cc and beta.numel() == Cc, "gamma/beta [C] fp32")
    _req(gamma.is_contiguous() and beta.is_contiguous(), "gamma/beta contiguous")
    for o, dt in ((out16, F16), (out32, F32)):
        if o is not None:
            _req(o.dtype == dt and o.shape == x.shape and o.stride(1) == 1, "bad LN output tensor")
    for m in (mod_scale, mod_shift):
        if m is not None:
            _req(m.dtype == F32 and m.numel() == Cc and m.is_contiguous(), "modulation vectors must be fp32 [C]")
    _aligned(16, x=x, gamma=gamma, beta=beta, out32=out32, mod_scale=mod_scale, mod_shift=mod_shift)
    _aligned(8, out16=out16)
    lib = _lib.load()
    check(lib.cut3r_layernorm(_p(x), x.stride(0), _p(gamma), _p(beta), float(eps), M, Cc,
                              _p(out16), out16.stride(0) if out16 is not None else 0,
                              _p(out32), out32.stride(0) if out32 is not None else 0,
                              _p(mod_scale), _p(mod_shift), _stream()), "cut3r_layernorm")


def layernorm_dual(x, g1, b1, out1, g2, b2, out2, eps=1e-6):
    _cuda(x, g1, b1, out1, g2, b2, out2)
    M, Cc = x.shape
    _req(x.dtype == F32 and x.stride(1) == 1 and Cc in (768, 1024, 1536), "x fp32 [M,C], C in {768,1024,1536}")
    for o in (out1, out2):
        _req(o.dtype == F16 and o.shape == (M, Cc) and o.stride(1) == 1, "outputs fp16 [M,C]")
    for t in (g1, b1, g2, b2):
        _req(t.dtype == F32 and t.numel() == Cc and t.is_contiguous(), "gamma/beta fp32 [C]")
    _req(float(eps) > 0.0, f"layernorm_dual: eps must be > 0, got {eps}")
    _aligned(16, x=x, g1=g1, b1=b1, g2=g2, b2=b2)
    _aligned(8, out1=out1, out2=out2)
    lib = _lib.load()
    check(lib.cut3r_layernorm_dual(_p(x), x.stride(0), _p(g1), _p(b1), _p(out1), out1.stride(0), _p(g2), _p(b2), _p(out2), out2.stride(0),
                                   float(eps), M, Cc, _stream()), "cut3r_layernorm_dual")


def layernorm_tokens(x, gamma, beta, eps, pose32, pose16, tok16, tok32=None):
    _cuda(x, gamma, beta, pose32, pose16, tok16, tok32)
    _req(x.dtype == F32 and x.dim() == 2 and x.stride(1) == 1, "x must be fp32 [M,C] with unit inner stride")
    _req(tok16.dim() == 3, "tok16 [Wn,N,C]")
    Wn, N, Cc = tok16.shape
    _req(Wn > 0 and N > 0 and x.shape == (Wn * (N + 1), Cc), f"x must hold Wn * (N + 1) = {Wn * (N + 1)} rows of {Cc}")
    _req(gamma.dtype == F32 and beta.dtype == F32 and gamma.numel() == Cc and beta.numel() == Cc, "gamma/beta [C] fp32")
    _req(gamma.is_contiguous() and beta.is_contiguous(), "gamma/beta contiguous")
    _req(float(eps) > 0.0, f"layernorm_tokens: eps must be > 0, got {eps}")
    for o, dt in ((pose32, F32), (pose16, F16)):
        _req(o.dtype == dt and o.shape == (Wn, Cc) and o.stride(1) == 1, "pose outputs [Wn,C] with unit inner stride")
    for o, dt in ((tok16, F16), (tok32, F32)):
        if o is not None:
            _req(o.dtype == dt and o.shape == (Wn, N, Cc) and o.stride(2) == 1 and o.stride(1) == Cc, "token outputs [Wn,N,C], rows of a group contiguous")
    _aligned(16, x=x, gamma=gamma, beta=beta, pose32=pose32, tok32=tok32)
    _aligned(8, pose16=pose16, tok16=tok16)
    lib = _lib.load()
    check(lib.cut3r_layernorm_tokens(_p(x), x.stride(0), _p(gamma), _p(beta), float(eps), Wn, N, Cc, _p(pose32), pose32.stride(0),
                                     _p(pose16), pose16.stride(0), _p(tok16), tok16.stride(0), _p(tok32),
                                     tok32.stride(0) if tok32 is not None else 0, _stream()), "cut3r_layernorm_tokens")


LN_FOLD_MAX_K = 1024
GEMM_STAGES = int(os.environ.get("CUT3R_GEMM_STAGES", "0"))


def _fill_common(d, A, Bw, out, bias, res1, res2, act, tile):
    d.A, d.B, d.C = A.data_ptr(), Bw.data_ptr(), out.data_ptr()
    d.bias = bias.data_ptr() if bias is not None else None
    d.act = act
    d.out_f16 = 1 if out.dtype == F16 else 0
    d.batch = 1
    d.tile = tile
    d.stages = GEMM_STAGES
    for i, r in ((1, res1), (2, res2)):
        if r is not None:
            _req(r.dtype in (F16, F32) and r.stride(-1) == 1, "residual must be fp16/fp32 with unit inner stride")
            setattr(d, f"res{i}", r.data_ptr())
            setattr(d, f"ldr{i}", r.stride(-2))
            setattr(d, f"res{i}_f16", 1 if r.dtype == F16 else 0)


_ROPE_TABLES = {}
ROPE_PMIN, ROPE_NPOS = -1, 258


def rope_table(device, base, fwd=1.0, head_dim=64):
    key = (str(device), float(base), float(fwd), int(head_dim))
    t = _ROPE_TABLES.get(key)
    if t is None:
        t = torch.empty(2, ROPE_NPOS, head_dim // 4, dtype=F32, device=device)
        lib = _lib.load()
        check(lib.cut3r_rope2d_table(_p(t), ROPE_PMIN, ROPE_NPOS, head_dim // 4, float(base), float(fwd), _stream()), "cut3r_rope2d_table")
        _ROPE_TABLES[key] = t
    return t


def _launch(d, what):
    check(_lib.load().cut3r_gemm_f16(C.byref(d), _stream()), what)


def _linear_desc(A, W, out, bias, act, res1, tile, rope=None, ln=None, emit=None, *, res2=None, pair=False):
    _cuda(A, W, out, bias, res1, res2)
    _req(A.dtype == F16 and W.dtype == F16 and A.dim() == 2 and W.dim() == 2, "A,W must be 2-D fp16")
    M, K = A.shape
    N = W.shape[0]
    _req(W.shape[1] == K and out.shape == (M, N), f"shape mismatch A{tuple(A.shape)} W{tuple(W.shape)} out{tuple(out.shape)}")
    _req(A.stride(1) == 1 and W.stride(1) == 1 and out.stride(1) == 1, "unit inner strides required")
    _req(out.dtype in (F16, F32), "out must be fp16 or fp32")
    if bias is not None:
        _req(bias.dtype == F32 and bias.numel() == N and bias.is_contiguous(), "bias fp32 [N]")
    for r in (res1, res2):
        if r is not None:
            _req(r.shape == (M, N), "residual shape")
    d = GemmDesc()
    if rope is not None:
        pos, cols, base = rope[:3]
        hd = rope[3] if len(rope) > 3 else 64
        _req(pos.dtype == torch.int64 and pos.is_contiguous() and pos.numel() == 2 * M and pos.is_cuda, "rope positions int64 [M,2]")
        _req(out.dtype == F16 and act == 0 and res1 is None and res2 is None and (hd == 64 or (hd == 48 and not pair)) and cols % hd == 0
             and 0 < cols <= N and N % hd == 0 and tile != 16, "fused rope: fp16 output, no activation / residual, whole heads of 64 or 48")
        tab = rope_table(out.device, base, 1.0, hd)
        d.rope_pos, d.rope_table, d.rope_cols, d.rope_pmin, d.rope_npos, d.rope_d = pos.data_ptr(), tab.data_ptr(), int(cols), ROPE_PMIN, ROPE_NPOS, hd
    _fill_common(d, A, W, out, bias, res1, res2, act, tile)
    d.M, d.N, d.K, d.lda, d.ldb, d.ldc = M, N, K, A.stride(0), W.stride(0), out.stride(0)
    if ln is not None:
        st, cs, eps = ln
        _cuda(st, cs)
        _req(K <= LN_FOLD_MAX_K, f"LayerNorm fold: K = {K} > {LN_FOLD_MAX_K}, the widest row the folded epilogue normalises (run ops.layernorm in front instead)")
        _req(K % 64 == 0 and st.dtype == F32 and st.is_contiguous() and st.numel() == M * (K // 64) * 2, f"ln stats fp32 [K/64={K // 64}, M={M}, 2]")
        _req(cs.dtype == F32 and cs.is_contiguous() and cs.numel() == N and bias is not None and tile != 16, "ln colsum fp32 [N], folded bias required")
        d.ln_stats, d.ln_colsum, d.ln_nslab, d.ln_eps = st.data_ptr(), cs.data_ptr(), K // 64, float(eps)
    if emit is not None:
        so, o16 = emit
        _cuda(so, o16)
        _req(N % 64 == 0 and so.dtype == F32 and so.is_contiguous() and so.numel() == M * (N // 64) * 2, f"stats_out fp32 [N/64={N // 64}, M={M}, 2]")
        _req(o16.dtype == F16 and o16.shape == (M, N) and o16.stride(1) == 1, "out16 fp16 [M,N]")
        _req(out.dtype == F32 and res1 is not None and res1.dtype == F32 and res2 is None and act == 0 and tile != 16, "emit: fp32 output with an fp32 residual")
        d.stats_out, d.out16, d.ld16 = so.data_ptr(), o16.data_ptr(), o16.stride(0)
    return d


def linear(A, W, out, bias=None, act=0, res1=None, res2=None, tile=0, rope=None, ln=None, emit=None):
# ... 1301 lines not shown
```

cut3r_slam_amd/track_backend.py:

```python
from __future__ import annotations

import math

import numpy as np
import torch

from . import geom_host as gh
from . import ops
from .lietorch import SE3, Sim3


class TrackBackend:
    def __init__(self, slam, keyframes, config, device="cuda:0"):
        self.device = device
        self.keyframes = keyframes
        self.model = slam.model
        self.graph = slam.graph
        self.loop_iters = int(config.get("iteration", 0))
        self.loop_group = str(config.get("loop_group", "se3"))
        if self.loop_group not in ops.LC_GROUPS:
            raise ValueError(f"loop_group: one of {sorted(ops.LC_GROUPS)}, not {self.loop_group!r}")
        self._chain_ws = None
        self.downsample_ratio = slam.downsample_ratio
        self.conf_th = 0.05
        self.lc_initialized = False
        self.closed_loop = {"idx_current": [], "idx_matched": [], "pointmaps_lc": []}
        self._lsum = torch.zeros(1, dtype=torch.float64, device=device)
        self._count = torch.zeros(1, dtype=torch.int32, device=device)
        self._ws = None

    def _feat_overlap(self, f0, f1s, thr=0.7):
        N, C = f0.shape
        need = 2 * (N - 1) * C + N
        if self._ws is None or self._ws.numel() < need:
            self._ws = torch.empty(need, device=self.device)
        B = len(f1s)
        if B == 1:
            counts = torch.zeros(1, dtype=torch.int32, device=self.device)
            ops.patch_overlap_count(f0.contiguous(), f1s[0].contiguous(), thr, self._ws, counts)
            return counts.float() / float(N - 1)
        feats = torch.stack([f.contiguous() for f in f1s], 0)
        need = (B + 1) * (N - 1) * C + N
        if self._chain_ws is None or self._chain_ws[0].numel() < need or self._chain_ws[1].numel() < 2 * B + 1:
            self._chain_ws = (torch.empty(need, device=self.device), torch.zeros(2 * B + 1, dtype=torch.int32, device=self.device))
        ws, ints = self._chain_ws
        ops.patch_overlap_chain(f0.contiguous(), feats, thr, -1.0, None, ws, ints[2 * B:2 * B + 1], ints[:B], ints[B:2 * B])
        return ints[:B].float() / float(N - 1)

    def nms_scores(self, ids_matched, idx_current, K4):
        kf = self.keyframes
        h, w = kf.submap_ds.shape[2], kf.submap_ds.shape[3]
        if kf.feat_rows:
            raise RuntimeError("loop closure needs the full keyframe feature store (KeyFrame feat_buffer = 0)")
        ids = torch.as_tensor(np.asarray(ids_matched), dtype=torch.long)
        pm_matched = kf.submap_ds[ids // 5, ids % 5].contiguous()
        pm_cur = kf.submap_ds[idx_current // 5, idx_current % 5].contiguous()
        B = len(ids)
        a2c = torch.empty(B, dtype=torch.int32, device=self.device)
        c2a = torch.empty(B, dtype=torch.int32, device=self.device)
        ops.overlap_bwd(pm_matched, kf.w2c[idx_current].contiguous(), K4, w, h, a2c)
        ops.overlap_fwd(pm_cur, kf.w2c[ids.to(kf.w2c.device)].contiguous(), K4, w, h, c2a, clamp_z=False)
        feat = self._feat_overlap(kf.featI[idx_current], [kf.featI[int(i)] for i in ids])
        overlap = (a2c.float() / (h * w) + c2a.float() / (h * w)) / 2
        return (0.8 * overlap + 0.2 * feat).cpu()

    def nms(self, ids_matched, idx_current, K4, th=0.4):
        scores = self.nms_scores(ids_matched, idx_current, K4)
        if float(scores.max()) > th:
            return int(torch.argmax(scores))
        return None

    def track(self, selected_idx, anchor_sub_num):
        kf, ds = self.keyframes, self.downsample_ratio
        sel = torch.as_tensor(np.asarray(selected_idx), dtype=torch.long)
        sel_d = sel.to(kf.image.device)
        miss = [int(i) for i in sel if not kf.feat_valid[int(i)]]
        if miss:
            mi = torch.as_tensor(miss, device=kf.image.device)
            kf.featI[mi] = self.model.encode_batch(kf.image[mi])
            for i in miss:
                kf.feat_valid[i] = True
        preds, _ = self.model.decode_window(kf.featI[sel_d].contiguous(), kf.ht, kf.wd)
        pts = torch.cat([p["pts3d_in_self_view"] for p in preds], 0).contiguous()
        conf = torch.cat([p["conf_self"] for p in preds], 0).contiguous()
        enc = torch.cat([p["camera_pose"] for p in preds], 0)
        V, H, W, _ = pts.shape
        a = anchor_sub_num * 5
        ops.logdepth_sum(kf.depth[a], pts[0], self._lsum)
        host = enc.detach().cpu().numpy()
        align_s = np.float32(math.exp(np.float32(float(self._lsum.item()) / (H * W))))
        poses = gh.pose_encoding_to_camera(host)
        first_w2c = gh.inv4(poses[0])
        prev = gh.pose_vec_to_matrix(kf.pose[a].numpy()[None])[0]
        pm = torch.empty(V, H // ds, W // ds, 3, device=self.device)
        cf = torch.empty(V, H // ds, W // ds, device=self.device)
        dp = torch.empty(H, W, device=self.device)
        out_poses = []
        for i in range(V):
            pose = gh.chain_pose(first_w2c, poses[i], prev[:3, :3], prev[:3, 3], align_s)
            ops.align_view(pts[i], conf[i], pose[:3, :4].reshape(-1), float(align_s), ds, pm[i], cf[i], dp)
            out_poses.append(gh.matrix_to_pose_vec(pose))
        return pm, cf, np.stack(out_poses)

    def _rewrite(self, sub0, sub1, T34, include_last=True):
        kf = self.keyframes
        B = sub1 - sub0 + 1
        block = kf.submap_ds[sub0:sub1 + 1]
        ops.transform_submaps(block, T34.reshape(B, 12).contiguous())
        Th = T34.detach().cpu().numpy()
        i0, n = sub0 * 5, B * 5 + (1 if include_last else 0)
        c2w = gh.pose_vec_to_matrix(kf.pose[i0:i0 + n].numpy())
        if self.loop_group == "sim3":
            row = np.minimum(np.arange(n) // 5, B - 1)
            out, s = gh.similarity_on_poses(Th[row], c2w)
            ops.scale_planes(kf.depth[i0:i0 + n], torch.from_numpy(s.astype(np.float32)).to(kf.depth.device))
            new = gh.matrices_to_pose_vecs(out)
            kf.set_poses(i0, new)
            return new
        out = np.empty_like(c2w)
        for j in range(n):
            Ts = np.eye(4, dtype=np.float32)
            Ts[:3, :4] = Th[min(j // 5, B - 1)]
            out[j] = Ts @ c2w[j]
        new = gh.matrices_to_pose_vecs(out)
        kf.set_poses(i0, new)
        return new

    def loop_closure_init(self, pointmap_current_lc, idx_matched, idx_current, return_loss=False):
        kf = self.keyframes
        sub0, sub1 = 0, idx_current // 5
        block = kf.submap_ds[sub0:sub1 + 1]
        B = block.shape[0]
        mask = (kf.conf_ds[sub0:sub1, 5] > 0).reshape(B - 1, -1) if B > 1 else None
        cur = kf.submap_ds[sub1, idx_current % 5]
        res = ops.lc_optimize(block.contiguous(), mask, cur, pointmap_current_lc, self.loop_iters, 5e-4, return_loss, group=self.loop_group)
        xi, T = res[0], res[1]
        se3 = Sim3.exp(xi) if self.loop_group == "sim3" else SE3.exp(xi)
        new_pose = self._rewrite(sub0, sub1, T)
        updates = {"pose_updates": se3.data, "submap_idx": range(sub0, sub1 + 1),
                   "camera_idx": range(sub0 * 5, (sub1 + 1) * 5 + 1), "camera_pose": torch.from_numpy(new_pose)}
        if return_loss:
            updates["loss"] = res[2]
        return updates

    def loop_closure(self, pointmaps_lc, idx_matched, idx_current, return_loss=False):
        kf = self.keyframes
        sub1 = idx_current // 5
        block = kf.submap_ds[0:sub1 + 1]
        B, N6, h, w, _ = block.shape
        N = h * w
        prev_cur = np.array(self.closed_loop["idx_current"], dtype=np.int64)
        sub_cur_all = np.append(prev_cur // 5, sub1)
        pm_cur = torch.cat([kf.submap_ds[torch.as_tensor(prev_cur // 5), torch.as_tensor(prev_cur % 5)],
                            kf.submap_ds[sub1, idx_current % 5][None]], 0).contiguous()
        lc_all = torch.cat([torch.stack(self.closed_loop["pointmaps_lc"], 0), pointmaps_lc[None]], 0).float().contiguous()
        Bc = lc_all.shape[0]
        sub_matched_all = np.append(np.array(self.closed_loop["idx_matched"], dtype=np.int64) // 5, idx_matched // 5)
        terms = []
        w_fl = 1.0 / (3.0 * (B - 1) * N) if B > 1 else 0.0
        w_c = 1.0 / (3.0 * Bc * N)
        for p in range(B - 1):
            terms.append((block[p, N6 - 1], p, block[p + 1, 0], p + 1, w_fl, None))
        for k in range(Bc):
            terms.append((lc_all[k, 0], B + k, block[int(sub_matched_all[k]), 0], int(sub_matched_all[k]), w_c, None))
# ... 51 lines not shown
```

cut3r_slam_amd/track_frontend.py:

```python
from __future__ import annotations

import math
import time
import warnings

import numpy as np
import torch

from . import geom_host as gh
from . import ops
from .factor_graph import AlignedPoints, SubmapStore
from .self_calib import SelfCalibration


def _check_scale(t0, s, stats=None):
    s = float(s)
    if stats is not None:
        stats["windows"] += 1
        if math.isfinite(s) and s > 0:
            ls = math.log(s)
            stats["log_scale_last"] = ls
            stats["log_scale_absmax"] = max(stats["log_scale_absmax"], abs(ls))
    if not (math.isfinite(s) and s > 0):
        if stats is not None:
            stats["nonfinite_windows"] += 1
            if stats["first_nonfinite_keyframe"] is None:
                stats["first_nonfinite_keyframe"] = t0
        grew = stats is not None and stats["log_scale_absmax"] > 40.0
        warnings.warn(f"window at keyframe {t0}: chained log-depth scale is {s} ("
                      + ("the chained scale grew geometrically along the stream: |log s| reached "
                         f"{stats['log_scale_absmax']:.1f} before leaving the fp32 range" if grew else
                         "a non-positive or non-finite predicted depth in the shared keyframe, or an overflowing chained scale")
                      + "); poses from this window on are not finite", RuntimeWarning, stacklevel=3)


def new_scale_stats():
    return {"windows": 0, "nonfinite_windows": 0, "first_nonfinite_keyframe": None, "log_scale_last": 0.0, "log_scale_absmax": 0.0}


def make_views(model, images_u8):
    images = model.normalize(images_u8.float())
    views = []
    for i in range(len(images)):
        views.append({
            "img": images[i][None],
            "ray_map": torch.full((1, 6, images[i].shape[-2], images[i].shape[-1]), torch.nan),
            "true_shape": torch.from_numpy(np.int32([images[i].shape[-2], images[i].shape[-1]])),
            "idx": i, "instance": str(i),
            "camera_pose": torch.from_numpy(np.eye(4, dtype=np.float32)).unsqueeze(0),
            "img_mask": torch.tensor(True).unsqueeze(0), "ray_mask": torch.tensor(False).unsqueeze(0),
            "update": torch.tensor(True).unsqueeze(0), "reset": torch.tensor(False).unsqueeze(0)})
    return views


TIMING = {"sync1_s": 0.0, "sync2_s": 0.0, "windows": 0}


class TrackFrontend:
    def __init__(self, slam, keyframes, config, device="cuda:0"):
        self.device = device
        self.keyframes = keyframes
        self.model = slam.model
        self.graph = slam.graph
        self.t1 = 0
        self.warmup = 6
        self.frontend_nms = config.get("frontend_nms", 1)
        self.keyframe_thresh = config.get("keyframe_thresh", 4.0)
        self.frontend_window = config.get("frontend_window", 25)
        self.frontend_thresh = config.get("frontend_thresh", 16.0)
        self.frontend_radius = config.get("frontend_radius", 2)
        self.keyframes.mono_depth_alpha = config.get("mono_depth_alpha", 0.01)
        self.downsample_ratio = slam.downsample_ratio
        self.window_batch = int(config.get("window_batch", 1))
        self.sequence_windows = int(config.get("sequence_windows", 0))
        self._lsum = torch.zeros(1, dtype=torch.float64, device=device)
        self._lsum_host = torch.zeros(1, dtype=torch.float64).pin_memory()
        self._counts = None
        self._counts_host = None
        self._pose_host = torch.zeros(8, 7, dtype=torch.float32).pin_memory()
        self._ev = None
        self.scale_stats = new_scale_stats()
        self.calibration = SelfCalibration(getattr(slam, "config", None))
        self.on_calibrated = None

    def prepare_input(self, images):
        return make_views(self.model, images)

    def window_features(self, t0, t1):
        kf = self.keyframes
        missing = [i for i in range(t0, t1) if not kf.feat_valid[i]]
        if missing:
            runs, a = [], missing[0]
            for p, q in zip(missing, missing[1:] + [None]):
                if q != p + 1:
                    runs.append((a, p + 1))
                    a = q
            imgs = kf.image[runs[0][0]:runs[0][1]] if len(runs) == 1 else torch.cat([kf.image[a:b] for a, b in runs], 0)
            feats = self.model.encode_batch(imgs)
            o = 0
            for a, b in runs:
                kf.feat_store(a, b, feats[o:o + b - a])
                o += b - a
        return kf.feat_slice(t0, t1) if (not kf.feat_rows or t1 - t0 <= 6) else None

    def infer(self, imgs_u8=None, t0=None, t1=None):
        if t0 is not None:
            H, W = self.keyframes.ht, self.keyframes.wd
            preds, _ = self.model.decode_window(self.window_features(t0, t1), H, W)
        else:
            preds, _ = self.model.forward_window(imgs_u8)
        pts = torch.cat([p["pts3d_in_self_view"] for p in preds], 0)
        conf = torch.cat([p["conf_self"] for p in preds], 0)
        pose_enc = torch.cat([p["camera_pose"] for p in preds], 0)
        return pts.contiguous(), conf.contiguous(), pose_enc

    def predict(self, new_img, kf_img, kf_pose, kf_depth, kf_pointmap=None, outputs=None):
        ds = self.downsample_ratio
        if outputs is None:
            outputs = self.infer(torch.stack([kf_img, new_img], 0).to(self.device))
        pts, conf, pose_enc = outputs
        _, H, W, _ = pts.shape
        kf_depth = torch.as_tensor(kf_depth).to(self.device, torch.float32).contiguous()
        lsum = torch.zeros(1, dtype=torch.float64, device=self.device)
        ops.logdepth_sum(kf_depth, pts[0].contiguous(), lsum)
        packed = torch.cat([pose_enc.detach().reshape(-1).double(), lsum]).cpu().numpy()
        host, lsum = packed[:-1].astype(np.float32).reshape(2, 7), float(packed[-1])
        poses = gh.pose_encoding_to_camera(host)
        align_s = np.float32(math.exp(np.float32(lsum / (H * W))))
        _check_scale("of predict()", align_s)
        prev_c2w = gh.pose_vec_to_matrix(np.asarray(torch.as_tensor(kf_pose).cpu(), np.float32)[None])[0]
        pose = gh.chain_pose(gh.inv4(poses[0]), poses[1], prev_c2w[:3, :3], prev_c2w[:3, 3], align_s)
        pm = torch.empty(H // ds, W // ds, 3, device=self.device)
        cf = torch.empty(H // ds, W // ds, device=self.device)
        depth = torch.empty(H, W, device=self.device)
        ops.align_view(pts[1].contiguous(), conf[1].contiguous(), pose[:3, :4].reshape(-1), float(align_s), ds, pm, cf, depth)
        new_pose = torch.from_numpy(gh.matrix_to_pose_vec(pose))
        return new_pose, depth, pm, conf[0][::ds, ::ds].contiguous()

    def track(self, t0, t1, init=False, outputs=None):
        if outputs is None:
            outputs = self.infer(t0=t0, t1=t1)
        self.track_many([(t0, t1)], [outputs], init=init)

    def seq_base(self, t0):
        S = 5 * self.sequence_windows
        return (t0 // S) * S if S > 0 else 0

    def _decide(self, t0, t1, init, done, base=0):
        graph = self.graph
        if init:
            if base != graph.base:
                graph.begin_sequence(base)
            graph.add_neighborhood_factors(0, 3, r=3)
        for i in range(t0, t1):
            if not init:
                graph.add_neighborhood_factors(i - 3, i + 1, r=3)
            if i in done:
                graph.add_finish(*done[i])

    def prefetch_logdepth(self, t0, pts, pose_enc):
        kf = self.keyframes
        if pose_enc.is_cuda:
            self._pose_host[:pose_enc.shape[0]].copy_(pose_enc.detach(), non_blocking=True)
        ops.logdepth_accum(kf.depth[t0], pts[0], self._lsum)
        self._lsum_host.copy_(self._lsum, non_blocking=True)
        ev = torch.cuda.Event()
        ev.record()
        return ev

    def track_many(self, ranges, outputs, init=False, first_event=None, count_mask=None, exchange=None, defer_decisions=False):
        kf, graph, ds = self.keyframes, self.graph, self.downsample_ratio
        deferred = [] if exchange is not None else None
        L = ((max(t1 - self.seq_base(t0) for t0, t1 in ranges) + 63) // 64) * 64
        all_counts = torch.zeros(len(ranges), 6, 2, L, dtype=torch.int32) if exchange is not None else None
        if self._ev is None:
            self._ev = torch.cuda.Event()
        pending = None
        lsum_next = None
        h, w = kf.submap_ds.shape[2:4]
        for k, ((t0, t1), (pts, conf, pose_enc)) in enumerate(zip(ranges, outputs)):
            V, H, W, _ = pts.shape
            b0 = self.seq_base(t0)
            init_k = init or (b0 == t0 and t0 > 0)
            if k == 0 and first_event is not None and not init_k:
                tic = time.perf_counter()
# ... 138 lines not shown

        bases = [self.seq_base(t0) for t0, _ in ranges]
        cut = [b0 == t0 and t0 > 0 for b0, (t0, _) in zip(bases, ranges)]

        def scale_of(k):
            if cut[k]:
                chain["log_s"], chain["L5"] = 0.0, float(scal[k, 1])
                return np.float32(1.0)
            lsum = chain["log_s"] * (H * W) + chain["L5"] - float(scal[k, 0])
            align_s = np.float32(math.exp(np.float32(lsum / (H * W))))
            chain["log_s"], chain["L5"] = math.log(float(align_s)), float(scal[k, 1])
            return align_s

        encs = scal[:, 2:2 + 7 * V].reshape(n, V, 7).astype(np.float32)
        chained_all, s_all, vecs, rows_all = gh.chain_windows(encs, scale_of, kf.pose[ranges[0][0]].numpy(), reset=cut)
        for k in range(n):
            if not cut[k]:
                _check_scale(ranges[k][0], s_all[k], self.scale_stats)
        cent = []
        for k, (t0, t1) in enumerate(ranges):
            kf.pose[t0:t1] = torch.from_numpy(vecs[k])
            cent.append(kf.pose[bases[k]:t1, :3].numpy().copy())
        per = [(chained_all[k], s_all[k], rows_all[k]) for k in range(n)]
        ta, tb = ranges[0][0], ranges[-1][1]
        allrows = np.zeros((tb - ta, 12), np.float32)
        for (t0, t1), (_, _, rows) in zip(ranges, per):
            allrows[t0 - ta:t1 - ta] = rows
        if getattr(self, "_rows_pinned", None) is None or self._rows_pinned.shape[0] < tb - ta:
            self._rows_pinned = torch.zeros(max(64, tb - ta), 12).pin_memory()
        self._rows_pinned[:tb - ta].copy_(torch.from_numpy(allrows))
        kf.w2c[ta:tb].copy_(self._rows_pinned[:tb - ta], non_blocking=True)
        L = ((max(t1 - b0 for (t0, t1), b0 in zip(ranges, bases)) + 63) // 64) * 64
        nown = i1 - i0
        cm = getattr(self, "_counts_many", None)
        if cm is None or cm.shape[0] < nown or cm.shape[-1] < L:
            self._counts_many = torch.zeros(nown, 6, 2, max(256, 2 * L), dtype=torch.int32, device=self.device)
            self._counts_many_host = torch.zeros(tuple(self._counts_many.shape), dtype=torch.int32).pin_memory()
        intr_all = kf.intrinsic[ta:tb].numpy()

        def update(k, counting):
            (t0, t1), (pts, conf, _), (chained, s_win, rows) = ranges[k], outs_own[k - i0], per[k]
            V = t1 - t0
            intr = intr_all[t0 - ta:t1 - ta]
            if not all(np.array_equal(intr[v], intr[0]) for v in range(V)):
                raise NotImplementedError("sharded tracking assumes one calibration per window")
            sub, b0 = t0 // 5, bases[k]
            ops.window_update(pts, conf, np.concatenate([c[:3, :4].reshape(-1) for c in chained]), float(s_win), ds,
                              kf.submap_ds[sub, :V], kf.conf_ds[sub, :V], kf.depth[t0:t1], kf.submap_ds[b0 // 5:], kf.w2c[b0:], t0 - b0,
                              3 if counting else (1 << 30), [float(x) for x in intr[0]], self._counts_many[k - i0, :V], w2c_new=rows.reshape(-1))

        for k in range(i0, i1):
            update(k, False)
        gather_store(ranges[0][0] // 5, n, 0)
        all_counts = torch.zeros(n, 6, 2, L, dtype=torch.int32)
        if self._ev is None:
            self._ev = torch.cuda.Event()
        for k in range(i0, i1):
            update(k, True)
        kf.w2c[ta:tb].copy_(self._rows_pinned[:tb - ta], non_blocking=True)
        gather_store(ranges[0][0] // 5, n, 1)
        self._counts_many_host[:nown].copy_(self._counts_many[:nown], non_blocking=True)
        self._ev.record()
        self._ev.synchronize()
        for k in range(i0, i1):
            t0, t1 = ranges[k]
            all_counts[k, :t1 - t0, :, :t1 - bases[k]] = self._counts_many_host[k - i0, :t1 - t0, :, :t1 - bases[k]]
        total = exchange_counts(all_counts).numpy()

        def finish():
            for k, (t0, t1) in enumerate(ranges):
                b0 = bases[k]
                if cut[k]:
                    if b0 != graph.base:
                        graph.begin_sequence(b0)
                    graph.add_neighborhood_factors(0, 3, r=3)
                graph.window_decide(t0 - b0, t1 - b0, cent[k], total[k, :t1 - t0], H * W, h * w, cut[k])
        if defer_decisions:
            return finish
        finish()
        return None

    def track_batch(self, ranges, after_window=None):
        kf = self.keyframes
        self.window_features(ranges[0][0], ranges[-1][1])
        feats = torch.stack([self.window_features(a, b) for a, b in ranges], 0)
        res = self.model.decode_windows(feats, kf.ht, kf.wd)
        V = ranges[0][1] - ranges[0][0]
        outs = [(res["pts3d_in_self_view"][j * V:(j + 1) * V], res["conf_self"][j * V:(j + 1) * V], res["camera_pose"][j * V:(j + 1) * V])
                for j in range(len(ranges))]
        if after_window is None:
            self.track_many(ranges, outs)
            self.t1 = ranges[-1][1]
            return
        for rng, out in zip(ranges, outs):
            self.track_many([rng], [out])
            self.t1 = rng[1]
            after_window(rng[0], rng[1])

    def run(self, tstamp, last_frame=False, after_window=None):
        kf = self.keyframes
        if not kf.is_initialized and kf.counter.value - 1 == self.warmup:
            t1 = kf.counter.value - 1
            self.track(0, t1, init=True)
            kf.is_initialized = True
            self.t1 = t1
            return False, range(0, t1), 0
        elif kf.is_initialized and self.window_batch > 1:
            Wb = self.window_batch
            if self.t1 < kf.counter.value - 5 * Wb:
                first = self.t1 - 1
                self.track_batch([(first + 5 * j, first + 5 * j + 6) for j in range(Wb)], after_window=after_window)
                t1 = self.t1
                return (t1 > 10) and after_window is None, range(first, t1), (t1 - 6) // 5
            if last_frame:
                while self.t1 < kf.counter.value - 1:
                    t0 = self.t1 - 1
                    t1 = min(t0 + 6, kf.counter.value - 1)
                    self.track(t0, t1)
                    self.t1 = t1
                    if after_window is not None and t1 == t0 + 6 and t1 <= kf.counter.value - 2:
                        after_window(t0, t1)
                return False, None, None
            return False, None, None
        elif kf.is_initialized and self.t1 < kf.counter.value - 5:
            t0 = self.t1 - 1
            t1 = kf.counter.value - 1
            self.track(t0, t1)
            self.t1 = t1
            return (t1 > 10), range(t0, t1), t0 // 5
        elif last_frame and kf.is_initialized:
            t0 = self.t1 - 1
            t1 = kf.counter.value - 1
            if t1 > t0:
                self.track(t0, t1)
                self.t1 = t1
            return False, range(t0, t1), t0 // 5
        return False, None, None
```

include/cut3r_hip.h:

```cpp
#ifndef CUT3R_HIP_H
#define CUT3R_HIP_H
#include <stdint.h>
#ifdef __cplusplus
extern "C" {
#endif

int cut3r_abi_version(void);

int cut3r_rope2d(void* tokens, int dtype, const int64_t* positions, int B, int N, int H, int D,
                 long long sB, long long sN, long long sH, float base, float fwd, void* stream);
int cut3r_rope2d_qk(void* q, void* k, int dtype, const int64_t* positions, int B, int N, int H, int D, long long q_sB,
                    long long q_sN, long long k_sB, long long k_sN, float base, float fwd, void* stream);

int cut3r_rope2d_tab(void* t0, const int64_t* pos0, long long ntok0, long long stride0, void* t1, const int64_t* pos1, long long ntok1,
                     long long stride1, int H, int D, const float* table, int pmin, int npos, float base, float fwd, void* stream);

int cut3r_layernorm(const float* x, int ldx, const float* gamma, const float* beta, float eps, int M, int C,
                    void* y16, int ld16, float* y32, int ld32, const float* mod_scale, const float* mod_shift,
                    void* stream);
int cut3r_layernorm_dual(const float* x, int ldx, const float* g1, const float* b1, void* y1, int ld1, const float* g2,
                         const float* b2, void* y2, int ld2, float eps, int M, int C, void* stream);
int cut3r_layernorm_tokens(const float* x, int ldx, const float* gamma, const float* beta, float eps, int Wn, int N, int C,
                           float* pose32, long long pose32_gs, void* pose16, long long pose16_gs, void* tok16, long long tok16_gs,
                           float* tok32, long long tok32_gs, void* stream);

typedef struct cut3r_gemm_desc {
    const void* A;
    const void* B;
    void* C;
    const float* bias;
    const void* res1;
    const void* res2;
    int M, N, K, lda, ldb, ldc, ldr1, ldr2;
    int act;
    int out_f16, res1_f16, res2_f16;
    int batch;
    long long strideA, strideB, strideC, strideBias, strideR1, strideR2;
    int conv_k;
    int H, W, Cin, conv_stride, Ho, Wo;
    int relu_in;
    int shuf;
    int shuf_cout, shuf_Hin, shuf_Win;
    int tile;
    int stages;
    const void* rope_pos;
    const float* rope_table;
    int rope_cols, rope_pmin, rope_npos;
    int rope_d;
    const float* ln_stats;
    const float* ln_colsum;
    int ln_nslab;
    float ln_eps;
    float* stats_out;
    void* out16;
    int ld16;
} cut3r_gemm_desc;
int cut3r_gemm_f16(const cut3r_gemm_desc* d, void* stream);
int cut3r_rope2d_table(float* table, int pmin, int npos, int Q, float base, float fwd, void* stream);
int cut3r_gemm_tile_for(const cut3r_gemm_desc* d);
int cut3r_gemm_f16_pair(const cut3r_gemm_desc* d0, const cut3r_gemm_desc* d1, void* stream);
int cut3r_gemm_kernel_for(const cut3r_gemm_desc* d);
int cut3r_gemm_pair_kernel_for(const cut3r_gemm_desc* d0, const cut3r_gemm_desc* d1);
int cut3r_gemm_kernel_count(void);

int cut3r_gemv_f16w(const float* X, int ldx, const void* W, int ldw, const float* bias, float* Y, int ldy,
                    int M, int N, int K, int act, const float* res, int ldr, int silu_in, void* stream);

int cut3r_attention_f16(const void* q, const void* k, const void* v, void* out, int B, int H, int Nq, int Nk, int D,
                        long long q_sb, long long q_sn, long long k_sb, long long k_sn, long long v_sb, long long v_sn,
                        long long o_sb, long long o_sn, float scale, void* stream);

int cut3r_attention_one_key_f16(const void* v, void* out, int B, int H, int Nq, int D, long long v_sb, long long v_sn, long long o_sb,
                                long long o_sn, void* stream);

int cut3r_attention_variant(int v);
int cut3r_attention_kernel_for(int B, int H, int Nq, int D);

int cut3r_im2col_patch(const void* img, int u8, int B, int C, int H, int W, int P, void* out, void* stream);
int cut3r_cast_f32_f16(const float* x, int ldx, void* y, int ldy, int M, int C, void* stream);
int cut3r_colmean(const float* x, int ldx, int M, int C, float* y, void* stream);
int cut3r_colmean_batched(const float* x, int B, long long stride_x, int ldx, int M, int C, float* y, long long stride_y, void* stream);

int cut3r_upsample2x_nhwc(const void* in, void* out, int B, int H, int W, int C, void* stream);
int cut3r_dpt_final(const void* in, int P, int Cin, const float* w, const float* b, int mode, float* pts, float* conf,
                    void* stream);
int cut3r_conv3x3_dpt_final(const cut3r_gemm_desc* d, const float* w, const float* b, int mode, float* pts, long long pts_view_stride,
                            float* conf, long long conf_view_stride, void* stream);
int cut3r_postprocess_pts(const float* raw, int P, int nch, int pos_z, float* pts, float* conf, void* stream);
int cut3r_postprocess_pose(const float* raw, int B, float* out, void* stream);

int cut3r_patch_overlap(const float* feat0, const float* feat1, int N, int C, float thr, void* ws, int32_t* count,
                        void* stream);
int cut3r_patch_overlap_chain(const float* feat_last, const float* feats, int B, int N, int C, float thr_sim, double thr_ratio,
                              const int32_t* forced_host, void* ws, int32_t* state, int32_t* counts, int32_t* decisions,
                              void* stream);

int cut3r_overlap_fwd(const float* pm, int N, const float* P_host, float s_align, const float* w2c, int B, float fx, float fy,
                      float cx, float cy, int W, int H, int clamp_z ,
                      int32_t* counts, void* stream);
int cut3r_overlap_bwd(const float* pms, int B, int N, int grp, int grp_stride, const float* w2c, float fx, float fy, float cx,
                      float cy, int W, int H, int32_t* counts, void* stream);

int cut3r_window_update(const float* pts, const float* conf, int V, int H, int W, const float* P_host, float s, int ds,
                        float* pm_ds, float* conf_ds, float* depth, const float* store, int grp, int grp_stride,
                        float* w2c, const float* w2c_new_host, int t0, int first, float fx, float fy, float cx, float cy,
                        int32_t* counts, int ldc, double* lsum_reset, void* stream);

int cut3r_logdepth_accum(const float* prev_depth, const float* pts, int n, double* out, void* stream);

int cut3r_align_view(const float* pts, const float* conf, int H, int W, const float* P_host, float s, int ds,
                     float* pm_ds, float* conf_ds, float* depth, void* stream);
int cut3r_logdepth_sum(const float* prev_depth, const float* pts, int n, double* out, void* stream);

int cut3r_lie_unary(int group, int op, const float* in, float* out, int n, void* stream);
int cut3r_lie_unary_bwd(int group, int op, const float* in, const float* grad_out, float* grad_in, int n, void* stream);
int cut3r_lie_mul(int group, const float* x, const float* y, float* out, int n, void* stream);
int cut3r_lie_mul_bwd(int group, const float* x, const float* y, const float* grad_out, float* grad_x, float* grad_y, int n,
                      void* stream);
int cut3r_lie_act(int group, const float* x, const float* p, float* out, int n, int P, int pd, void* stream);
int cut3r_lie_act_bwd(int group, const float* x, const float* p, const float* grad_out, float* grad_x, float* grad_p, int n, int P,
                      int pd, void* stream);
int cut3r_lie_adj(int group, const float* x, const float* a, float* out, int n, int transpose, void* stream);

int cut3r_lc_workspace_floats(int B, int N);
int cut3r_lc_optimize(const float* first, const float* last, long long sub_stride, const unsigned char* mask, const float* cur,
                      const float* cur_lc, int B, int N, long long n_masked, int iters, float lr, float* xi, float* adam_m,
                      float* adam_v, float* T, float* workspace, float* loss_out, void* stream);
typedef struct cut3r_lc_term {
    const float* a;
    const float* c;
    const unsigned char* mask;
    int ia, ic;
    float w;
    int pad;
} cut3r_lc_term;
int cut3r_lc_optimize_terms(const void* terms_dev, int n_terms, int P, int N, int iters, float lr, float* xi, float* adam_m,
                            float* adam_v, float* T, float* workspace, float* loss_out, void* stream);
int cut3r_lc_optimize_sim3(const float* first, const float* last, long long sub_stride, const unsigned char* mask, const float* cur,
                           const float* cur_lc, int B, int N, long long n_masked, int iters, float lr, float* xi, float* adam_m,
                           float* adam_v, float* T, float* workspace, float* loss_out, void* stream);
int cut3r_lc_optimize_terms_sim3(const void* terms_dev, int n_terms, int P, int N, int iters, float lr, float* xi, float* adam_m,
                                 float* adam_v, float* T, float* workspace, float* loss_out, void* stream);
int cut3r_transform_submaps(float* pts, const float* T, int B, long long points_per_submap, void* stream);
int cut3r_scale_planes(float* planes, const float* scale, int n, long long per_plane, void* stream);

int cut3r_corr_index_forward(const float* volume, const float* coords, float* out, int BN, int h1, int w1, int h2, int w2,
                             int radius, void* stream);
int cut3r_corr_index_backward(const float* coords, const float* grad_out, float* grad_volume, int BN, int h1, int w1, int h2, int w2,
                              int radius, void* stream);
long long cut3r_ba_workspace_floats(int P, int ht, int wd, int N, int M, int fixedp);
int cut3r_ba_step(const float* Gij, const float* disps, const float* intr, const float* target, const float* weight, const float* eta,
                  const int* ii, const int* jj, const int* src_ptr, const int* src_edges, const int* kx, const unsigned char* present,
                  int P, int ht, int wd, int N, int M, int fixedp, float ep, float lm, float* workspace, float* dx, float* dz, int* flag,
                  void* stream);
int cut3r_ba_assemble(const float* Gij, const float* disps, const float* intr, const float* target, const float* weight, const float* eta,
                      const int* ii, const int* jj, const int* src_ptr, const int* src_edges, const int* kx, const unsigned char* present,
                      int P, int ht, int wd, int N, int M, int fixedp, int motion_only, float* workspace, float* S_out, float* vS_out,
                      float* hdiag_out, void* stream);
int cut3r_ba_solve(const float* S, const float* vS, const float* hdiag, int n, float ep, float lm, float* scratch, float* dx, int* flag,
                   void* stream);
int cut3r_ba_backsub(float* workspace, const float* dx, const unsigned char* present, int P, int ht, int wd, int N, int M, int fixedp,
                     float* dz, void* stream);
int cut3r_ba_proj_trans(const float* Gij, const float* disps, const float* intr, const float* target, const float* weight, const int* ii,
                        const int* jj, const int* src_ptr, const int* src_edges, const int* kx, int P, int ht, int wd, int N, int M,
// ... 211 lines not shown
```

Before: 5848.

## Write encoder features in place into fp16/mean rings and gather windows on GPU

Adds an in-place path where the final encoder layernorm writes straight into slot-indexed fp32 and fp16 feature rings. A per-slot column-mean ring is kept alongside, and decoder windows are assembled by a slot-driven gather kernel. This replaces the Python-side ring stores, the torch.stack of window features and the repeated fp32-to-fp16 casts and mean computations at decode time. It adds extra ring memory, pinned host slot lists with event syncs, and an early gather in the sharded tracker, and it is enabled by default through CUT3R_FEAT_INPLACE.

```diff
diff --git a/cut3r_slam_amd/_lib.py b/cut3r_slam_amd/_lib.py
--- a/cut3r_slam_amd/_lib.py
+++ b/cut3r_slam_amd/_lib.py
@@ -46,6 +46,10 @@
                              c_int, c_void_p],
     "cut3r_layernorm_tokens": [c_void_p, c_int, c_void_p, c_void_p, c_float, c_int, c_int, c_int, c_void_p, c_ll, c_void_p, c_ll, c_void_p,
                                c_ll, c_void_p, c_ll, c_void_p],
+    "cut3r_layernorm_slots": [c_void_p, c_int, c_void_p, c_void_p, c_float, c_int, c_int, c_int, c_void_p, c_void_p, c_int, c_void_p,
+                              c_void_p, c_void_p],
+    "cut3r_colmean_slots": [c_void_p, c_int, c_int, c_void_p, c_void_p, c_int, c_int, c_void_p, c_void_p],
+    "cut3r_window_gather": [c_void_p, c_void_p, c_void_p, c_int, c_int, c_int, c_int, c_void_p, c_void_p, c_void_p],
     "cut3r_gemm_f16": [C.POINTER(GemmDesc), c_void_p],
     "cut3r_gemm_tile_for": [C.POINTER(GemmDesc)],
     "cut3r_gemm_f16_pair": [C.POINTER(GemmDesc), C.POINTER(GemmDesc), c_void_p],
diff --git a/cut3r_slam_amd/csrc/elementwise.hip b/cut3r_slam_amd/csrc/elementwise.hip
--- a/cut3r_slam_amd/csrc/elementwise.hip
+++ b/cut3r_slam_amd/csrc/elementwise.hip
@@ -264,6 +264,27 @@
 }
 
 template <int NV>
+__global__ __launch_bounds__(256) void layernorm_slots_kernel(const float* __restrict__ x, int ldx, const float* __restrict__ gamma,
+                                                              const float* __restrict__ beta, float eps, int M, int C, int N,
+                                                              const int* __restrict__ slot, const int* __restrict__ slot2, int rows,
+                                                              float* __restrict__ d32, h16* __restrict__ d16) {
+    const int lane = threadIdx.x & 63;
+    const int row = blockIdx.x * 4 + (threadIdx.x >> 6);
+    if (row >= M) return;
+    const int b = row / N, n = row - b * N;
+    const float* xr = x + (size_t)row * ldx;
+    const int s[2] = {slot[b], slot2[b]};
+    if ((unsigned)s[0] >= (unsigned)rows) return;
+#pragma unroll
+    for (int k = 0; k < 2; k++) {
+        if ((unsigned)s[k] >= (unsigned)rows) continue;
+        const size_t off = ((size_t)s[k] * N + n) * C;
+        if constexpr (NV > 0) layernorm_fast_row<NV>(xr, gamma, beta, eps, lane, d16 + off, d32 + off, nullptr, nullptr);
+        else layernorm_row(xr, gamma, beta, eps, C, lane, d16 + off, d32 + off, nullptr, nullptr);
+    }
+}
+
+template <int NV>
 __global__ __launch_bounds__(256) void layernorm_dual_kernel(const float* __restrict__ x, int ldx, const float* __restrict__ g1,
                                                              const float* __restrict__ b1, h16* __restrict__ y1, int ld1,
                                                              const float* __restrict__ g2, const float* __restrict__ b2,
@@ -344,11 +365,8 @@
     }
 }
 
-__global__ __launch_bounds__(256) void colmean_kernel(const float* __restrict__ x, int ldx, int M, int C, float* __restrict__ y,
-                                                      long long sx, long long sy) {
+DEVINL void colmean_block(const float* __restrict__ x, int ldx, int M, int C, float* __restrict__ y, float* __restrict__ y2) {
     __shared__ float part[16][64];
-    x += (size_t)blockIdx.y * sx;
-    y += (size_t)blockIdx.y * sy;
     const int col = threadIdx.x & 63, rg = threadIdx.x >> 6;
     const int c = blockIdx.x * 64 + col;
     float s0 = 0.f, s1 = 0.f, s2 = 0.f, s3 = 0.f;
@@ -364,7 +382,45 @@
     }
     part[rg][col] = (s0 + s1) + (s2 + s3);
     __syncthreads();
-    if (rg == 0 && c < C) y[c] = (part[0][col] + part[1][col] + part[2][col] + part[3][col]) / (float)M;
+    if (rg == 0 && c < C) {
+        const float mean = (part[0][col] + part[1][col] + part[2][col] + part[3][col]) / (float)M;
+        y[c] = mean;
+        if (y2) y2[c] = mean;
+    }
+}
+
+__global__ __launch_bounds__(256) void colmean_kernel(const float* __restrict__ x, int ldx, int M, int C, float* __restrict__ y,
+                                                      long long sx, long long sy) {
+    colmean_block(x + (size_t)blockIdx.y * sx, ldx, M, C, y + (size_t)blockIdx.y * sy, nullptr);
+}
+
+__global__ __launch_bounds__(256) void colmean_slots_kernel(const float* __restrict__ ring, int N, int C, const int* __restrict__ slot,
+                                                            const int* __restrict__ slot2, int rows, float* __restrict__ g) {
+    const int s = slot[blockIdx.y], s2 = slot2[blockIdx.y];
+    if ((unsigned)s >= (unsigned)rows) return;
+    colmean_block(ring + (size_t)s * N * C, C, N, C, g + (size_t)s * C, (unsigned)s2 < (unsigned)rows ? g + (size_t)s2 * C : nullptr);
+}
+
+__global__ __launch_bounds__(256) void window_gather_kernel(const h16* __restrict__ ring16, const float* __restrict__ ringg,
+                                                            const int* __restrict__ slots, int rows, int per16, int E4,
+                                                            h16* __restrict__ out16, float* __restrict__ outg) {
+    const int j = blockIdx.y;
+    const int s = slots[j];
+    if ((unsigned)s >= (unsigned)rows) return;
+    const half8_t* src = reinterpret_cast<const half8_t*>(ring16) + (size_t)s * per16;
+    half8_t* dst = reinterpret_cast<half8_t*>(out16) + (size_t)j * per16;
+    const int step = gridDim.x * 256;
+    int i = blockIdx.x * 256 + threadIdx.x;
+    for (; i + 3 * step < per16; i += 4 * step) {
+        const half8_t a = src[i], b = src[i + step], c = src[i + 2 * step], d = src[i + 3 * step];
+        dst[i] = a; dst[i + step] = b; dst[i + 2 * step] = c; dst[i + 3 * step] = d;
+    }
+    for (; i < per16; i += step) dst[i] = src[i];
+    if (blockIdx.x == 0) {
+        const f32x4* gs = reinterpret_cast<const f32x4*>(ringg) + (size_t)s * E4;
+        f32x4* gd = reinterpret_cast<f32x4*>(outg) + (size_t)j * E4;
+        for (int e = threadIdx.x; e < E4; e += 256) gd[e] = gs[e];
+    }
 }
 
 __global__ __launch_bounds__(256) void upsample2x_kernel(const h16* __restrict__ in, h16* __restrict__ out, int B, int H, int W, int C8) {
@@ -696,6 +752,24 @@
     return cut3r_check_launch();
 }
 
+extern "C" int cut3r_layernorm_slots(const float* x, int ldx, const float* gamma, const float* beta, float eps, int B, int N, int C,
+                                     const int32_t* slot, const int32_t* slot2, int rows, float* dst32, void* dst16, void* stream) {
+    if (!x || !gamma || !beta || !slot || !slot2 || !dst32 || !dst16) return CUT3R_ERR_ARG;
+    if (B <= 0 || N <= 0 || rows <= 0 || C <= 0 || (C & 3) || C > 2048 || ldx < C || (ldx & 3) || !(eps > 0.f)) return CUT3R_ERR_ARG;
+    if ((long long)B * N > 0x7fffffffLL || (long long)rows * N > 0x7fffffffLL) return CUT3R_ERR_ARG;
+    if (misaligned(x, 15) || misaligned(gamma, 15) || misaligned(beta, 15) || misaligned(dst32, 15) || misaligned(dst16, 7) ||
+        misaligned(slot, 3) || misaligned(slot2, 3))
+        return CUT3R_ERR_ARG;
+    const int M = B * N;
+    hipStream_t s = (hipStream_t)stream;
+    dim3 grid((M + 3) / 4), block(256);
+    if (C == 768) hipLaunchKernelGGL((layernorm_slots_kernel<3>), grid, block, 0, s, x, ldx, gamma, beta, eps, M, C, N, slot, slot2, rows, dst32, (h16*)dst16);
+    else if (C == 1024) hipLaunchKernelGGL((layernorm_slots_kernel<4>), grid, block, 0, s, x, ldx, gamma, beta, eps, M, C, N, slot, slot2, rows, dst32, (h16*)dst16);
+    else if (C == 1536) hipLaunchKernelGGL((layernorm_slots_kernel<6>), grid, block, 0, s, x, ldx, gamma, beta, eps, M, C, N, slot, slot2, rows, dst32, (h16*)dst16);
+    else hipLaunchKernelGGL((layernorm_slots_kernel<0>), grid, block, 0, s, x, ldx, gamma, beta, eps, M, C, N, slot, slot2, rows, dst32, (h16*)dst16);
+    return cut3r_check_launch();
+}
+
 extern "C" int cut3r_im2col_patch(const void* img, int u8, int B, int C, int H, int W, int P, void* out, void* stream) {
     if (!img || !out || B <= 0 || C <= 0 || P <= 0 || (P & 7) || H % P || W % P) return CUT3R_ERR_ARG;
     const size_t total = (size_t)B * (H / P) * (W / P) * (C * P * P / 8);
@@ -722,6 +796,29 @@
                                      void* stream) {
     if (!x || !y || B <= 0 || B > 65535 || M <= 0 || C <= 0) return CUT3R_ERR_ARG;
     hipLaunchKernelGGL(colmean_kernel, dim3((C + 63) / 64, B), dim3(256), 0, (hipStream_t)stream, x, ldx, M, C, y, stride_x, stride_y);
+    return cut3r_check_launch();
+}
+
+extern "C" int cut3r_colmean_slots(const float* ring32, int N, int C, const int32_t* slot, const int32_t* slot2, int B, int rows,
+                                   float* ring_mean, void* stream) {
+    if (!ring32 || !slot || !slot2 || !ring_mean || B <= 0 || B > 65535 || N <= 0 || C <= 0 || rows <= 0) return CUT3R_ERR_ARG;
+    if (misaligned(slot, 3) || misaligned(slot2, 3)) return CUT3R_ERR_ARG;
+    hipLaunchKernelGGL(colmean_slots_kernel, dim3((C + 63) / 64, B), dim3(256), 0, (hipStream_t)stream, ring32, N, C, slot, slot2, rows, ring_mean);
+    return cut3r_check_launch();
+}
+
+extern "C" int cut3r_window_gather(const void* ring16, const float* ring_mean, const int32_t* slots, int nslot, int rows, int N, int E,
+                                   void* out16, float* out_mean, void* stream) {
+    if (!ring16 || !ring_mean || !slots || !out16 || !out_mean) return CUT3R_ERR_ARG;
+    if (nslot <= 0 || nslot > 65535 || rows <= 0 || N <= 0 || E <= 0 || (E & 7)) return CUT3R_ERR_ARG;
+    if ((long long)N * E / 8 > 0x3fffffffLL) return CUT3R_ERR_ARG;
+    if (misaligned(ring16, 15) || misaligned(ring_mean, 15) || misaligned(out16, 15) || misaligned(out_mean, 15) || misaligned(slots, 3))
+        return CUT3R_ERR_ARG;
+    const int per16 = (int)((long long)N * E / 8);
+    int gx = (per16 + 1023) / 1024;
+    if (gx > 1024) gx = 1024;
+    hipLaunchKernelGGL(window_gather_kernel, dim3(gx, nslot), dim3(256), 0, (hipStream_t)stream, (const h16*)ring16, ring_mean, slots, rows, per16,
+                       E / 4, (h16*)out16, out_mean);
     return cut3r_check_launch();
 }
 
diff --git a/cut3r_slam_amd/dist.py b/cut3r_slam_amd/dist.py
--- a/cut3r_slam_amd/dist.py
+++ b/cut3r_slam_amd/dist.py
@@ -46,6 +46,8 @@
         "conf_ds_f32": nsub * (win + 1) * h * w * 4,
         "w2c_f32": n_kf * 12 * 4,
         "encoder_feature_ring_f32": feat_rows * tokens * feat_dim * 4,
+        "encoder_feature_ring_f16": feat_rows * tokens * feat_dim * 2,
+        "encoder_feature_mean_ring_f32": feat_rows * feat_dim * 4,
         "camera_frames_u8": frames_resident * frame_bytes,
         "weights_f16": int(weights_bytes),
         "network_workspaces": int(workspace_bytes),
@@ -115,6 +117,17 @@
         return self.base[int(key) % self.period].to(self.device)
 
 
+class _StoreWindows:
+    is_cuda = True
+
+    def __init__(self, ranges):
+        self.ranges = list(ranges)
+        self.gathered = None
+
+    def record_stream(self, stream):
+        pass
+
+
 class ShardedTracker:
 
     def __init__(self, slam, world: int, rank: int, wb: int = 1, infer_fn: Callable = None, track_fn: Callable = None,
@@ -135,6 +148,7 @@
         self._appended_upto = 0
         self._enc_stream, self._ahead = None, None
         self.encode_ahead = os.environ.get("CUT3R_ENC_AHEAD", "1") == "1"
+        self.gather_early = True
         self.side_priority = int(os.environ.get("CUT3R_SIDE_PRIORITY", "0"))
         self.scan = world > 1 or force_collective or os.environ.get("CUT3R_SCAN", "0") == "1"
         self.replicate_depth = os.environ.get("CUT3R_REPLICATE_DEPTH", "0") == "1"
@@ -161,12 +175,23 @@
         tr = self.slam.tracker
         if self.world > 1:
             self.slam.keyframes.feat_valid[ranges[0][0]] = False
+        if getattr(self.slam.model, "feat_inplace", False):
+            tr.window_features(ranges[0][0], ranges[-1][1], in_place=True)
+            return _StoreWindows(ranges)
         tr.window_features(ranges[0][0], ranges[-1][1])
         return torch.stack([tr.window_features(a, b) for a, b in ranges], 0)
 
+    def _gather(self, feats):
+        if isinstance(feats, _StoreWindows) and feats.gathered is None:
+            feats.gathered = self.slam.model.gather_windows(self.slam.keyframes, feats.ranges)
+
     def _decode(self, feats):
         kf = self.slam.keyframes
-        res = self.slam.model.decode_windows(feats, kf.ht, kf.wd)
+        if isinstance(feats, _StoreWindows):
+            self._gather(feats)
+            res = self.slam.model.decode_windows_slots(kf, feats.ranges, kf.ht, kf.wd, gathered=feats.gathered)
+        else:
+            res = self.slam.model.decode_windows(feats, kf.ht, kf.wd)
         return tuple(res[k] for k in ("pts3d_in_self_view", "conf_self", "camera_pose"))
 
     def _side_ctx(self, gathered, ev):
@@ -339,6 +364,8 @@
                     torch.cuda.current_stream().wait_event(self._upload_ev)
                 feats = self._encode(mine)
             self._ahead = None
+            if self.gather_early:
+                self._gather(feats)
             self.stats["issue_s"] += time.perf_counter() - tic
             self.stats["issue_enc_s"] += time.perf_counter() - tic
             t_next = t + n_frames
diff --git a/cut3r_slam_amd/keyframe.py b/cut3r_slam_amd/keyframe.py
--- a/cut3r_slam_amd/keyframe.py
+++ b/cut3r_slam_amd/keyframe.py
@@ -52,11 +52,40 @@
         self.featI = torch.zeros(self.feat_rows + 6 if self.feat_rows else buffer, n, feat_dim, dtype=torch.float, device=dev)
         self.pos = torch.zeros(buffer if not self.feat_rows else 1, n, 2, dtype=torch.int64, device=dev)
         self.feat_valid = _FeatValid(buffer, self.feat_rows)
+        self.featI16 = None
+        self.featG = None
+
+    def feat_rings(self):
+        if self.featI16 is None:
+            rows, n, e = self.featI.shape
+            self.featI16 = torch.empty((rows, n, e), dtype=torch.float16, device=self.device)
+            self.featG = torch.empty((rows, e), dtype=torch.float, device=self.device)
+            self.feat_sync(0, rows)
+        return self.featI, self.featI16, self.featG
+
+    def feat_sync(self, r0: int, r1: int) -> None:
+        from . import ops
+        n, e = self.featI.shape[1:]
+        for c in range(r0, r1, 4096):
+            d = min(r1, c + 4096)
+            ops.cast_f16(self.featI[c:d].view((d - c) * n, e), self.featI16[c:d].view((d - c) * n, e))
+            ops.colmean_batched(self.featI[c:d], self.featG[c:d])
+
+    def feat_slots(self, idx):
+        R = self.feat_rows
+        if not R:
+            for i in idx:
+                if not 0 <= int(i) < self.buffer:
+                    raise IndexError(f"keyframe {i} outside the feature store of {self.buffer} rows")
+            return [int(i) for i in idx], [-1] * len(idx)
+        return [int(i) % R for i in idx], [R + int(i) % R if int(i) % R < 6 else -1 for i in idx]
 
     def feat_store(self, a: int, b: int, feats) -> None:
         R = self.feat_rows
+        sync = (lambda r0, r1: self.feat_sync(r0, r1)) if self.featI16 is not None else (lambda r0, r1: None)
         if not R:
             self.featI[a:b] = feats
+            sync(a, b)
         else:
             if b - a > R:
                 raise ValueError("feature ring smaller than one encoder batch")
@@ -65,9 +94,11 @@
                 r = i % R
                 m = min(b - i, R - r)
                 self.featI[r:r + m] = feats[i - a:i - a + m]
+                sync(r, r + m)
                 if r < 6:
                     k = min(m, 6 - r)
                     self.featI[R + r:R + r + k] = feats[i - a:i - a + k]
+                    sync(R + r, R + r + k)
                 i += m
         for i in range(a, b):
             self.feat_valid[i] = True
diff --git a/cut3r_slam_amd/model.py b/cut3r_slam_amd/model.py
--- a/cut3r_slam_amd/model.py
+++ b/cut3r_slam_amd/model.py
@@ -87,6 +87,27 @@
         self.Nx, self.Ny, self.D = self.x.x.shape[0] // self.B, self.y.x.shape[0] // self.B, self.C // self.heads
 
 
+class _SlotList:
+
+    def __init__(self, n, device, depth=4):
+        self.dev = torch.full((n,), -1, dtype=torch.int32, device=device)
+        self.host = [torch.zeros(n, dtype=torch.int32).pin_memory() for _ in range(depth)]
+        self.done = [None] * depth
+        self.turn = 0
+
+    def put(self, values):
+        k = self.turn
+        self.turn = (k + 1) % len(self.host)
+        if self.done[k] is not None:
+            self.done[k].synchronize()
+        self.host[k].numpy()[:] = values
+        self.dev.copy_(self.host[k], non_blocking=True)
+        if self.done[k] is None:
+            self.done[k] = torch.cuda.Event()
+        self.done[k].record()
+        return self.dev
+
+
 class Cut3rModel:
     def __init__(self, cfg: Cut3rConfig, state_dict: Dict[str, torch.Tensor], device="cuda:0", minimal: bool = False):
         self.cfg = cfg
@@ -113,6 +134,8 @@
         self.head_chunk = max(1, _env_int("CUT3R_HEAD_CHUNK", 28))
         self.one_key = _env_flag("CUT3R_ONE_KEY", True)
         self.ln_fold = _env_int("CUT3R_LN_FOLD", 1)
+        self.feat_inplace = _env_flag("CUT3R_FEAT_INPLACE", True)
+        self._slot_lists: Dict[tuple, "_SlotList"] = {}
         self._head_stream = None
         self._side = None
         self._head_side = None
@@ -364,7 +387,7 @@
         with self._encoder_turn():
             return self._encode_pass(img)
 
-    def _encode_pass(self, img: torch.Tensor):
+    def _encode_pass(self, img: torch.Tensor, rings=None):
         cfg = self.cfg
         B, _, H, W = img.shape
         P, E = cfg.patch_size, cfg.enc_embed_dim
@@ -394,16 +417,23 @@
             else:
                 self._ln(x, p + ".norm2", out16=ln16)
                 self._mlp(tag, ln16, p + ".mlp", x, x)
+        if rings is not None:
+            featI, featI16, featG, slot, slot2 = rings
+            ops.layernorm_slots(x, *self.w["enc_norm"], cfg.ln_eps, slot, slot2, featI, featI16)
+            ops.colmean_slots(featI, slot, slot2, featG)
+            return None
         feat = torch.empty((B, N, E), dtype=F32, device=self.device)
         feat16 = torch.empty((B, N, E), dtype=F16, device=self.device)
         self._ln(x, "enc_norm", out16=feat16.view(M, E), out32=feat.view(M, E))
         return feat, feat16, pos
 
-    def _graphed(self, kind, fn, inp):
+    def _graphed(self, kind, fn, inp, in_place=False):
         key = (kind, tuple(inp.shape), inp.dtype)
         ent = self._graphs.get(key)
+        if ent is not None and in_place and ent[1] is not inp:
+            raise ValueError("a graph replayed in place reads the buffer it was captured with")
         if ent is None:
-            static_in = inp.clone()
+            static_in = inp if in_place else inp.clone()
             cur = torch.cuda.current_stream()
             side = torch.cuda.Stream()
             side.wait_stream(cur)
@@ -425,7 +455,8 @@
             ent = (graph, static_in, out)
             self._graphs[key] = ent
         graph, static_in, out = ent
-        static_in.copy_(inp, non_blocking=True)
+        if not in_place:
+            static_in.copy_(inp, non_blocking=True)
         graph.replay()
         return out
 
@@ -665,6 +696,65 @@
                 return feat.clone()
         return self._encode(imgs)[0]
 
+    def _slot_list(self, key, n):
+        sl = self._slot_lists.get(key)
+        if sl is None:
+            sl = self._slot_lists[key] = _SlotList(n, self.device)
+        return sl
+
+    @torch.no_grad()
+    def encode_into(self, imgs: torch.Tensor, keyframes, a: int, b: int, index=None) -> None:
+        idx = list(range(a, b)) if index is None else [int(i) for i in index]
+        B = imgs.shape[0]
+        if len(idx) != B:
+            raise ValueError(f"{B} images for {len(idx)} keyframes")
+        if keyframes.feat_rows and B > keyframes.feat_rows:
+            raise ValueError("feature ring smaller than one encoder batch")
+        featI, featI16, featG = keyframes.feat_rings()
+        rows, N, E = featI.shape
+        P = self.cfg.patch_size
+        if (N, E) != ((imgs.shape[2] // P) * (imgs.shape[3] // P), self.cfg.enc_embed_dim) or featI.device != self.device:
+            raise ValueError("the keyframe store does not hold the features of images of this size")
+        slot, slot2 = keyframes.feat_slots(idx)
+        ops.check_slots(slot, rows)
+        ops.check_slots(slot2, rows, allow_negative=True)
+        key = (featI.data_ptr(), featI16.data_ptr(), featG.data_ptr(), rows)
+        with self._encoder_turn():
+            dev = self._slot_list(("enc", B) + key, 2 * B).put(slot + slot2)
+            rings = (featI, featI16, featG, dev[:B], dev[B:])
+            if self.use_graphs:
+                self._graphed(("encS",) + key, lambda x: self._encode_pass(x, rings), imgs.contiguous())
+            else:
+                self._encode_pass(imgs, rings)
+        for i in idx:
+            keyframes.feat_valid[i] = True
+
+    @torch.no_grad()
+    def gather_windows(self, keyframes, ranges):
+        _, featI16, featG = keyframes.feat_rings()
+        rows, N, E = featI16.shape
+        Wn, V = len(ranges), ranges[0][1] - ranges[0][0]
+        if Wn < 1 or V < 1 or any(t1 - t0 != V for t0, t1 in ranges) or (keyframes.feat_rows and V > 6):
+            raise ValueError("windows of one length (at most 6 keyframes from a ring)")
+        idx = [i for t0, t1 in ranges for i in range(t0, t1)]
+        missing = [i for i in idx if not keyframes.feat_valid[i]]
+        if missing:
+            raise ValueError(f"the keyframe store does not hold the features of keyframes {missing[:4]}")
+        slots = keyframes.feat_slots(idx)[0]
+        ops.check_slots(slots, rows)
+        feat16 = self.buf("decS.feat16", (Wn, V, N, E), F16)
+        g32 = self.buf("decS.g32", (Wn, V, E), F32)
+        dev = self._slot_list(("dec", Wn * V), Wn * V).put(slots)
+        ops.window_gather(featI16, featG, dev, feat16, g32)
+        return feat16, g32
+
+    @torch.no_grad()
+    def decode_windows_slots(self, keyframes, ranges, H: int, W: int, gathered=None):
+        feat16, g32 = gathered if gathered is not None else self.gather_windows(keyframes, ranges)
+        if self.use_graphs:
+            return self._graphed(("decWs", H, W), lambda f: self._decode(None, f, H, W, False, gmean=g32)[0], feat16, in_place=True)
+        return self._decode(None, feat16, H, W, False, gmean=g32)[0]
+
     @torch.no_grad()
     def decode_window(self, feats: torch.Tensor, H: int, W: int):
         if self.use_graphs:
@@ -690,10 +780,12 @@
             return self._graphed(("decW", H, W), lambda f: self._decode(f, None, H, W, False)[0], feats.contiguous())
         return self._decode(feats, None, H, W, False)[0]
 
-    def _decode(self, feat, feat16, H, W, return_taps=False):
+    def _decode(self, feat, feat16, H, W, return_taps=False, gmean=None):
         cfg = self.cfg
         P, E, D, Ld = cfg.patch_size, cfg.enc_embed_dim, cfg.dec_embed_dim, cfg.dec_depth
-        Wn, V, N, _ = feat.shape
+        if feat is None and (feat16 is None or gmean is None or return_taps):
+            raise ValueError("a decoder pass without the fp32 features needs their fp16 copy and column means (and has no taps)")
+        Wn, V, N, _ = (feat if feat is not None else feat16).shape
         nh, nw = H // P, W // P
         S = cfg.state_size
         dev = self.device
@@ -749,8 +841,9 @@
             head_pts = torch.empty((Wn * V, H, W, 3), dtype=F32, device=dev)
             head_conf = torch.empty((Wn * V, H, W), dtype=F32, device=dev)
         for i in range(V):
-            ops.colmean_batched(feat[:, i], g32)
-            ops.cast_f16(g32, g16)
+            if gmean is None:
+                ops.colmean_batched(feat[:, i], g32)
+            ops.cast_f16(g32 if gmean is None else gmean[:, i], g16)
             a, b = im[0], im[1]
             a3 = a.x.view(Wn, N + 1, D)
             if i == 0:
diff --git a/cut3r_slam_amd/ops.py b/cut3r_slam_amd/ops.py
--- a/cut3r_slam_amd/ops.py
+++ b/cut3r_slam_amd/ops.py
@@ -178,6 +178,67 @@
     check(lib.cut3r_layernorm_tokens(_p(x), x.stride(0), _p(gamma), _p(beta), float(eps), Wn, N, Cc, _p(pose32), pose32.stride(0),
                                      _p(pose16), pose16.stride(0), _p(tok16), tok16.stride(0), _p(tok32),
                                      tok32.stride(0) if tok32 is not None else 0, _stream()), "cut3r_layernorm_tokens")
+
+
+def _slot_list(name, t, n):
+    _req(t is not None and t.is_cuda and t.dtype == torch.int32 and t.dim() == 1 and t.numel() == n and t.is_contiguous(),
+         f"{name}: int32 [{n}] on the GPU")
+
+
+def check_slots(slots, rows, allow_negative=False):
+    for s in slots:
+        s = int(s)
+        _req((allow_negative and s < 0) or 0 <= s < rows, f"slot {s} outside the ring of {rows} rows")
+
+
+def layernorm_slots(x, gamma, beta, eps, slot, slot2, ring32, ring16):
+    _cuda(x, gamma, beta, ring32, ring16)
+    _req(x.dtype == F32 and x.dim() == 2 and x.stride(1) == 1, "x must be fp32 [M,C] with unit inner stride")
+    _req(ring32 is not None and ring16 is not None and ring32.dim() == 3 and ring32.dtype == F32 and ring16.dtype == F16 and
+         ring16.shape == ring32.shape and ring32.is_contiguous() and ring16.is_contiguous(), "rings: contiguous fp32 / fp16 [rows,N,C]")
+    rows, N, Cc = ring32.shape
+    _req(rows > 0 and N > 0 and x.shape[1] == Cc and x.shape[0] > 0 and x.shape[0] % N == 0, f"x must hold B * N rows of {Cc} (N = {N})")
+    B = x.shape[0] // N
+    _req(0 < Cc <= 2048 and Cc % 4 == 0, f"layernorm_slots: C must be a multiple of 4 up to 2048, got {Cc}")
+    _req(gamma.dtype == F32 and beta.dtype == F32 and gamma.numel() == Cc and beta.numel() == Cc, "gamma/beta [C] fp32")
+    _req(gamma.is_contiguous() and beta.is_contiguous(), "gamma/beta contiguous")
+    _req(float(eps) > 0.0, f"layernorm_slots: eps must be > 0, got {eps}")
+    _slot_list("slot", slot, B)
+    _slot_list("slot2", slot2, B)
+    _aligned(16, x=x, gamma=gamma, beta=beta, ring32=ring32)
+    _aligned(8, ring16=ring16)
+    lib = _lib.load()
+    check(lib.cut3r_layernorm_slots(_p(x), x.stride(0), _p(gamma), _p(beta), float(eps), B, N, Cc, _p(slot), _p(slot2), rows, _p(ring32),
+                                    _p(ring16), _stream()), "cut3r_layernorm_slots")
+
+
+def colmean_slots(ring32, slot, slot2, ring_mean):
+    _cuda(ring32, ring_mean)
+    _req(ring32 is not None and ring32.dtype == F32 and ring32.dim() == 3 and ring32.is_contiguous(), "ring32: contiguous fp32 [rows,N,C]")
+    rows, N, Cc = ring32.shape
+    _req(ring_mean is not None and ring_mean.dtype == F32 and ring_mean.shape == (rows, Cc) and ring_mean.is_contiguous(), "ring_mean: fp32 [rows,C]")
+    _req(slot is not None and slot.dim() == 1 and 0 < slot.numel() <= 65535, "slot: int32 [B], 0 < B <= 65535")
+    _slot_list("slot", slot, slot.numel())
+    _slot_list("slot2", slot2, slot.numel())
+    lib = _lib.load()
+    check(lib.cut3r_colmean_slots(_p(ring32), N, Cc, _p(slot), _p(slot2), slot.numel(), rows, _p(ring_mean), _stream()), "cut3r_colmean_slots")
+
+
+def window_gather(ring16, ring_mean, slots, out16, out_mean):
+    _cuda(ring16, ring_mean, out16, out_mean)
+    _req(ring16 is not None and ring16.dtype == F16 and ring16.dim() == 3 and ring16.is_contiguous(), "ring16: contiguous fp16 [rows,N,E]")
+    rows, N, E = ring16.shape
+    _req(ring_mean is not None and ring_mean.dtype == F32 and ring_mean.shape == (rows, E) and ring_mean.is_contiguous(), "ring_mean: fp32 [rows,E]")
+    _req(out16 is not None and out16.dtype == F16 and out16.dim() == 4 and out16.shape[2:] == (N, E) and out16.is_contiguous(), "out16: fp16 [Wn,V,N,E]")
+    Wn, V = out16.shape[:2]
+    _req(out_mean is not None and out_mean.dtype == F32 and out_mean.shape == (Wn, V, E) and out_mean.is_contiguous(), "out_mean: fp32 [Wn,V,E]")
+    _req(rows > 0 and N > 0 and E > 0 and E % 8 == 0, f"window_gather: E must be a multiple of 8, got {E}")
+    _req(0 < Wn * V <= 65535, "window_gather: 0 < Wn * V <= 65535")
+    _slot_list("slots", slots, Wn * V)
+    _aligned(16, ring16=ring16, ring_mean=ring_mean, out16=out16, out_mean=out_mean)
+    lib = _lib.load()
+    check(lib.cut3r_window_gather(_p(ring16), _p(ring_mean), _p(slots), Wn * V, rows, N, E, _p(out16), _p(out_mean), _stream()),
+          "cut3r_window_gather")
 
 
 LN_FOLD_MAX_K = 1024
diff --git a/cut3r_slam_amd/track_backend.py b/cut3r_slam_amd/track_backend.py
--- a/cut3r_slam_amd/track_backend.py
+++ b/cut3r_slam_amd/track_backend.py
@@ -80,6 +80,8 @@
             kf.featI[mi] = self.model.encode_batch(kf.image[mi])
             for i in miss:
                 kf.feat_valid[i] = True
+                if kf.featI16 is not None:
+                    kf.feat_sync(i, i + 1)
         preds, _ = self.model.decode_window(kf.featI[sel_d].contiguous(), kf.ht, kf.wd)
         pts = torch.cat([p["pts3d_in_self_view"] for p in preds], 0).contiguous()
         conf = torch.cat([p["conf_self"] for p in preds], 0).contiguous()
diff --git a/cut3r_slam_amd/track_frontend.py b/cut3r_slam_amd/track_frontend.py
--- a/cut3r_slam_amd/track_frontend.py
+++ b/cut3r_slam_amd/track_frontend.py
@@ -86,7 +86,7 @@
     def prepare_input(self, images):
         return make_views(self.model, images)
 
-    def window_features(self, t0, t1):
+    def window_features(self, t0, t1, in_place=False):
         kf = self.keyframes
         missing = [i for i in range(t0, t1) if not kf.feat_valid[i]]
         if missing:
@@ -96,11 +96,16 @@
                     runs.append((a, p + 1))
                     a = q
             imgs = kf.image[runs[0][0]:runs[0][1]] if len(runs) == 1 else torch.cat([kf.image[a:b] for a, b in runs], 0)
+            if in_place:
+                self.model.encode_into(imgs, kf, missing[0], missing[-1] + 1, index=missing)
+                return None
             feats = self.model.encode_batch(imgs)
             o = 0
             for a, b in runs:
                 kf.feat_store(a, b, feats[o:o + b - a])
                 o += b - a
+        if in_place:
+            return None
         return kf.feat_slice(t0, t1) if (not kf.feat_rows or t1 - t0 <= 6) else None
 
     def infer(self, imgs_u8=None, t0=None, t1=None):
@@ -405,9 +410,13 @@
 
     def track_batch(self, ranges, after_window=None):
         kf = self.keyframes
-        self.window_features(ranges[0][0], ranges[-1][1])
-        feats = torch.stack([self.window_features(a, b) for a, b in ranges], 0)
-        res = self.model.decode_windows(feats, kf.ht, kf.wd)
+        if getattr(self.model, "feat_inplace", False):
+            self.window_features(ranges[0][0], ranges[-1][1], in_place=True)
+            res = self.model.decode_windows_slots(kf, ranges, kf.ht, kf.wd)
+        else:
+            self.window_features(ranges[0][0], ranges[-1][1])
+            feats = torch.stack([self.window_features(a, b) for a, b in ranges], 0)
+            res = self.model.decode_windows(feats, kf.ht, kf.wd)
         V = ranges[0][1] - ranges[0][0]
         outs = [(res["pts3d_in_self_view"][j * V:(j + 1) * V], res["conf_self"][j * V:(j + 1) * V], res["camera_pose"][j * V:(j + 1) * V])
                 for j in range(len(ranges))]
diff --git a/include/cut3r_hip.h b/include/cut3r_hip.h
--- a/include/cut3r_hip.h
+++ b/include/cut3r_hip.h
@@ -23,6 +23,8 @@
 int cut3r_layernorm_tokens(const float* x, int ldx, const float* gamma, const float* beta, float eps, int Wn, int N, int C,
                            float* pose32, long long pose32_gs, void* pose16, long long pose16_gs, void* tok16, long long tok16_gs,
                            float* tok32, long long tok32_gs, void* stream);
+int cut3r_layernorm_slots(const float* x, int ldx, const float* gamma, const float* beta, float eps, int B, int N, int C,
+                          const int32_t* slot, const int32_t* slot2, int rows, float* dst32, void* dst16, void* stream);
 
 typedef struct cut3r_gemm_desc {
     const void* A;
@@ -80,6 +82,10 @@
 int cut3r_cast_f32_f16(const float* x, int ldx, void* y, int ldy, int M, int C, void* stream);
 int cut3r_colmean(const float* x, int ldx, int M, int C, float* y, void* stream);
 int cut3r_colmean_batched(const float* x, int B, long long stride_x, int ldx, int M, int C, float* y, long long stride_y, void* stream);
+int cut3r_colmean_slots(const float* ring32, int N, int C, const int32_t* slot, const int32_t* slot2, int B, int rows, float* ring_mean,
+                        void* stream);
+int cut3r_window_gather(const void* ring16, const float* ring_mean, const int32_t* slots, int nslot, int rows, int N, int E, void* out16,
+                        float* out_mean, void* stream);
 
 int cut3r_upsample2x_nhwc(const void* in, void* out, int B, int H, int W, int C, void* stream);
 int cut3r_dpt_final(const void* in, int P, int Cin, const float* w, const float* b, int mode, float* pts, float* conf,
```

Measured after the change: 5880, median of 6. No clear change (+0.6%).
